# SuwoongHeo/neurecon

Hardware: AMD Instinct MI355X
Metric: rays/sec (4096 rays x 128 samples, 8-layer x256 SDF MLP) (higher is better)
Workload: dtype f16x3

## Files before the change

### include/neurecon_hip.h

```cpp
#ifndef NEURECON_HIP_H
#define NEURECON_HIP_H

#include <stddef.h>
#include <stdint.h>

#ifdef __cplusplus
extern "C" {
#endif

#define NR_OK 0
#define NR_ERR_ARG (-1)
#define NR_ERR_UNSUPPORTED (-2)
#define NR_ERR_HIP (-3)
#define NR_ERR_WORKSPACE (-4)

#define NR_PREC_FP32 0
#define NR_PREC_F16X3 1

#define NR_UPSAMPLE_OFFICIAL 0
#define NR_UPSAMPLE_DIRECT_USE 1
#define NR_UPSAMPLE_DIRECT_MORE 2

int nr_version(void);
const char* nr_last_error(void);
// ... 17 lines not shown
typedef struct {
  int D;
  int W;
  int skip;
  int multires;
  int W_geo_feat;
  int precision;
  int siren;
} NrSdfDesc;

size_t nr_sdf_packed_bytes(const NrSdfDesc* d);
int nr_sdf_pack(const NrSdfDesc* d, const float* const* W, const float* const* b, void* packed, void* stream);
size_t nr_mlp_workspace_bytes(int with_backward);
int nr_sdf_forward(const NrSdfDesc* d, const void* packed, const float* pts, int64_t P, float* sdf, float* nabla,
                   float* feature, void* workspace, size_t workspace_bytes, void* stream);

typedef struct {
  int D;
  int W;
  int multires;
  int multires_view;
  int W_geo_feat;
  int precision;
  int no_view_dirs;
  int siren;
} NrRadDesc;

size_t nr_radiance_packed_bytes(const NrRadDesc* d);
int nr_radiance_pack(const NrRadDesc* d, const float* const* W, const float* const* b, void* packed, void* stream);
int nr_radiance_forward(const NrRadDesc* d, const void* packed, const float* x, const float* vdir, int64_t vdir_div,
                        const float* normals, const float* feature, int64_t P, float* rgb, void* stream);

typedef struct {
  const float* rays_o;
  const float* rays_d;
  int64_t n_rays;
  const NrSdfDesc* sdf;
  const void* sdf_packed;
  const NrRadDesc* rad;
  const void* rad_packed;
  float s;
  float obj_bounding_radius;
  float near_bypass;
  float far_bypass;
  int N_samples;
  int N_importance;
  int N_upsample_iters;
  int calc_normal;
  int white_bkgd;
  const float* t_coarse;
  const float* u_fine;
  float* rgb;
  float* depth;
  float* acc;
  float* normals;
  float* d_final;
  float* sdf_out;
  float* nablas_out;
  float* radiance_out;
  float* alpha_out;
  float* cdf_out;
  float* weights_out;
  const NrNerfDesc* nerf;
  const void* nerf_packed;
  int N_outside;
  const float* t_outside;
  float* sigma_out;
  float* radiance_bg_out;
  int upsample_algo;
  float fixed_s;
  int N_nograd_samples;
  const float* t_nograd;
  void* workspace;
  size_t workspace_bytes;
  const float* u_rand;
  const float* t_out_rand;
  const float* s_dev;
  int sample_only;
  float* d_all_out;
  int no_mid_skip;
  int no_defer;
  int64_t max_chunk_rays;
  size_t max_workspace_bytes;
} NrNeusArgs;

#define NR_DEFAULT_WORKSPACE_BYTES ((size_t)4 << 30)
#define NR_MIN_CHUNK_RAYS 4096

size_t nr_neus_workspace_bytes(const NrNeusArgs* a);
int nr_neus_render(const NrNeusArgs* a, void* stream);

typedef struct {
  const float* rays_o;
  const float* rays_d;
  int64_t n_rays;
  const NrSdfDesc* sdf;
  const void* sdf_packed;
  const NrRadDesc* rad;
  const void* rad_packed;
  float alpha_net, beta_net;
  float beta_plus_init;
  float eps;
  float near, far;
  float obj_bounding_radius;
  int use_sphere_bg;
  int N_samples, N_importance, max_upsample_steps, max_bisection_steps;
  int calc_normal, white_bkgd;
  const float* t_coarse;
  const float* t_init;
  const float* u_up;
  const float* u_fine;
  float* rgb;
  float* depth;
  float* acc;
  float* normals;
  float* d_vals;
  float* sdf_out;
  float* nablas_out;
  float* radiance_out;
  float* alpha_out;
  float* p_out;
  float* weights_out;
  float* sigma_out;
  float* beta_map;
  float* iter_usage;
  void* workspace;
  size_t workspace_bytes;
  int N_outside;
  const NrNerfDesc* nerf;
  const void* nerf_packed;
  const float* rs_out;
  float beta_plus_k;
  float* sigma_bg;
  float* radiance_bg;
  const float* u_rand;
  const float* u_out;
} NrVolsdfArgs;

size_t nr_volsdf_workspace_bytes(const NrVolsdfArgs* a);
int nr_volsdf_render(const NrVolsdfArgs* a, void* stream);

typedef struct {
  const float* rays_o;
  const float* rays_d;
  int64_t n_rays;
  int64_t rays_per_batch;
  const NrSdfDesc* sdf;
  const void* sdf_packed;
  const NrRadDesc* rad;
  const void* rad_packed;
  float logit_tau;
  float radius_of_interest;
  float interval;
  float too_close_threshold;
  float near_bypass, far_bypass;
  int N_steps, N_secant_steps, N_query, N_freespace;
  int normal_mode;
  int64_t rayschunk, netchunk;
  int calc_normal, white_bkgd;
  const float* t_march;
  const float* t_query;
  const float* t_free;
  float* rgb;
  float* depth;
  float* acc;
  float* normals;
  float* surface_points;
  uint8_t* mask_surface;
  float* depth_surface;
  float* radiance_out;
  float* sdf_out;
  float* nablas_out;
  float* alpha_out;
// ... 265 lines not shown
```

### neurecon_amd/_lib.py

```python
import ctypes
import os
import threading

import torch

HERE = os.path.dirname(os.path.abspath(__file__))
LIB_PATH = os.environ.get('NR_LIB', os.path.join(HERE, 'libnrhip.so'))

PREC_FP32 = 0
PREC_F16X3 = 1
UPSAMPLE = {'official_solution': 0, 'direct_use': 1, 'direct_more': 2}

_c_p = ctypes.c_void_p
_c_i = ctypes.c_int
_c_i64 = ctypes.c_int64
_c_f = ctypes.c_float
_c_d = ctypes.c_double
_c_sz = ctypes.c_size_t


class NrSdfDesc(ctypes.Structure):
    _fields_ = [('D', _c_i), ('W', _c_i), ('skip', _c_i), ('multires', _c_i), ('W_geo_feat', _c_i),
                ('precision', _c_i), ('siren', _c_i)]


class NrRadDesc(ctypes.Structure):
    _fields_ = [('D', _c_i), ('W', _c_i), ('multires', _c_i), ('multires_view', _c_i), ('W_geo_feat', _c_i),
                ('precision', _c_i), ('no_view_dirs', _c_i), ('siren', _c_i)]


class NrNerfDesc(ctypes.Structure):
    _fields_ = [('D', _c_i), ('W', _c_i), ('skip', _c_i), ('input_ch', _c_i), ('multires', _c_i),
                ('multires_view', _c_i), ('precision', _c_i)]


class NrNeusArgs(ctypes.Structure):
    _fields_ = [
        ('rays_o', _c_p), ('rays_d', _c_p), ('n_rays', _c_i64),
        ('sdf', ctypes.POINTER(NrSdfDesc)), ('sdf_packed', _c_p),
        ('rad', ctypes.POINTER(NrRadDesc)), ('rad_packed', _c_p),
        ('s', _c_f), ('obj_bounding_radius', _c_f), ('near_bypass', _c_f), ('far_bypass', _c_f),
        ('N_samples', _c_i), ('N_importance', _c_i), ('N_upsample_iters', _c_i), ('calc_normal', _c_i),
        ('white_bkgd', _c_i),
        ('t_coarse', _c_p), ('u_fine', _c_p),
        ('rgb', _c_p), ('depth', _c_p), ('acc', _c_p), ('normals', _c_p),
        ('d_final', _c_p), ('sdf_out', _c_p), ('nablas_out', _c_p), ('radiance_out', _c_p),
        ('alpha_out', _c_p), ('cdf_out', _c_p), ('weights_out', _c_p),
        ('nerf', ctypes.POINTER(NrNerfDesc)), ('nerf_packed', _c_p), ('N_outside', _c_i), ('t_outside', _c_p),
        ('sigma_out', _c_p), ('radiance_bg_out', _c_p),
        ('upsample_algo', _c_i), ('fixed_s', _c_f), ('N_nograd_samples', _c_i), ('t_nograd', _c_p),
        ('workspace', _c_p), ('workspace_bytes', _c_sz),
        ('u_rand', _c_p), ('t_out_rand', _c_p), ('s_dev', _c_p), ('sample_only', _c_i), ('d_all_out', _c_p),
        ('no_mid_skip', _c_i), ('no_defer', _c_i), ('max_chunk_rays', _c_i64), ('max_workspace_bytes', _c_sz),
    ]


class NrVolsdfArgs(ctypes.Structure):
    _fields_ = [
        ('rays_o', _c_p), ('rays_d', _c_p), ('n_rays', _c_i64),
        ('sdf', ctypes.POINTER(NrSdfDesc)), ('sdf_packed', _c_p),
        ('rad', ctypes.POINTER(NrRadDesc)), ('rad_packed', _c_p),
        ('alpha_net', _c_f), ('beta_net', _c_f), ('beta_plus_init', _c_f), ('eps', _c_f),
        ('near', _c_f), ('far', _c_f), ('obj_bounding_radius', _c_f), ('use_sphere_bg', _c_i),
        ('N_samples', _c_i), ('N_importance', _c_i), ('max_upsample_steps', _c_i), ('max_bisection_steps', _c_i),
        ('calc_normal', _c_i), ('white_bkgd', _c_i),
        ('t_coarse', _c_p), ('t_init', _c_p), ('u_up', _c_p), ('u_fine', _c_p),
        ('rgb', _c_p), ('depth', _c_p), ('acc', _c_p), ('normals', _c_p),
        ('d_vals', _c_p), ('sdf_out', _c_p), ('nablas_out', _c_p), ('radiance_out', _c_p),
        ('alpha_out', _c_p), ('p_out', _c_p), ('weights_out', _c_p), ('sigma_out', _c_p),
        ('beta_map', _c_p), ('iter_usage', _c_p),
        ('workspace', _c_p), ('workspace_bytes', _c_sz),
        ('N_outside', _c_i), ('nerf', ctypes.POINTER(NrNerfDesc)), ('nerf_packed', _c_p), ('rs_out', _c_p),
        ('beta_plus_k', _c_f), ('sigma_bg', _c_p), ('radiance_bg', _c_p), ('u_rand', _c_p), ('u_out', _c_p),
    ]


class NrUnisurfArgs(ctypes.Structure):
    _fields_ = [
        ('rays_o', _c_p), ('rays_d', _c_p), ('n_rays', _c_i64), ('rays_per_batch', _c_i64),
        ('sdf', ctypes.POINTER(NrSdfDesc)), ('sdf_packed', _c_p),
        ('rad', ctypes.POINTER(NrRadDesc)), ('rad_packed', _c_p),
        ('logit_tau', _c_f), ('radius_of_interest', _c_f), ('interval', _c_f), ('too_close_threshold', _c_f),
        ('near_bypass', _c_f), ('far_bypass', _c_f),
        ('N_steps', _c_i), ('N_secant_steps', _c_i), ('N_query', _c_i), ('N_freespace', _c_i),
        ('normal_mode', _c_i), ('rayschunk', _c_i64), ('netchunk', _c_i64),
        ('calc_normal', _c_i), ('white_bkgd', _c_i),
        ('t_march', _c_p), ('t_query', _c_p), ('t_free', _c_p),
        ('rgb', _c_p), ('depth', _c_p), ('acc', _c_p), ('normals', _c_p),
        ('surface_points', _c_p), ('mask_surface', _c_p), ('depth_surface', _c_p),
        ('radiance_out', _c_p), ('sdf_out', _c_p), ('nablas_out', _c_p), ('alpha_out', _c_p), ('weights_out', _c_p),
        ('workspace', _c_p), ('workspace_bytes', _c_sz),
        ('u_query', _c_p), ('u_free', _c_p),
        ('shard_ray0', _c_i64), ('shard_row_rays', _c_i64), ('window_ss', _c_p), ('window_reduce', _c_p),
        ('window_user', _c_p), ('no_secant', _c_i), ('d_all_out', _c_p), ('sample_only', _c_i),
        ('full_march', _c_i),
    ]


WINDOW_REDUCE = ctypes.CFUNCTYPE(_c_i, _c_p)

TG_NONE, TG_SOFTPLUS, TG_MUL, TG_SPADJ, TG_RELUMASK = 0, 1, 3, 4, 5
BLK_X1, BLK_X2, BLK_Y, BLK_YB, BLK_Y2, BLK_Y3, BLK_A, BLK_G, BLK_ZD = 1, 2, 4, 8, 16, 32, 64, 128, 256
WG_BLK_A0, WG_BLK_A1, WG_BLK_B0, WG_BLK_B1 = 1, 2, 4, 8
WN_MAX = 16
ADAM_MAX = 64


class NrTrainGemm(ctypes.Structure):
    _fields_ = [
        ('op', _c_p), ('P', _c_i64),
        ('x1', _c_p), ('ld1', _c_i64), ('n1', _c_i),
        ('x2', _c_p), ('ld2', _c_i64), ('n2', _c_i),
        ('use_bias', _c_i), ('mode', _c_i), ('yscale', _c_f),
        ('y', _c_p), ('ldy', _c_i64), ('yb', _c_p), ('ldyb', _c_i64),
        ('y2', _c_p), ('ldy2', _c_i64), ('y3', _c_p), ('ldy3', _c_i64),
        ('a', _c_p), ('lda', _c_i64), ('g', _c_p), ('ldg', _c_i64), ('zd', _c_p), ('ldzd', _c_i64),
        ('g_row', _c_i), ('dot', _c_p), ('dot_bias', _c_f),
        ('head', _c_p), ('head_bias', _c_p), ('head_out', _c_p), ('blocked', _c_i),
        ('g_scaled', _c_i),
    ]


class NrWgrad(ctypes.Structure):
    _fields_ = [
        ('P', _c_i64), ('npairs', _c_i), ('a', _c_p * 2), ('lda', _c_i64 * 2), ('b', _c_p * 2), ('ldb', _c_i64 * 2),
        ('m', _c_i), ('n', _c_i), ('scale', _c_f), ('c', _c_p), ('ldc', _c_i64), ('colsum', _c_p),
        ('avec', _c_p), ('ldv', _c_i64), ('vec', _c_p), ('vec_scale', _c_f), ('workspace', _c_p),
        ('workspace_bytes', _c_sz), ('blocked', _c_i), ('fp32', _c_i),
    ]


class NrWnLayer(ctypes.Structure):
    _fields_ = [('v', _c_p), ('g', _c_p), ('w', _c_p), ('norm', _c_p), ('grad_w', _c_p), ('grad_v', _c_p),
                ('grad_g', _c_p), ('rows', _c_i), ('cols', _c_i)]


class NrAdamTensor(ctypes.Structure):
    _fields_ = [('param', _c_p), ('grad', _c_p), ('exp_avg', _c_p), ('exp_avg_sq', _c_p), ('n', _c_i64)]


class NrKernelStat(ctypes.Structure):
    _fields_ = [('name', ctypes.c_char * 32), ('launches', _c_i64), ('ms', ctypes.c_double),
                ('units', ctypes.c_double)]


_SIGS = {
    'nr_version': (_c_i, []),
    'nr_last_error': (ctypes.c_char_p, []),
    'nr_build_id': (ctypes.c_char_p, []),
    'nr_sdf_packed_bytes': (_c_sz, [ctypes.POINTER(NrSdfDesc)]),
    'nr_sdf_pack': (_c_i, [ctypes.POINTER(NrSdfDesc), ctypes.POINTER(_c_p), ctypes.POINTER(_c_p), _c_p, _c_p]),
    'nr_mlp_workspace_bytes': (_c_sz, [_c_i]),
    'nr_sdf_forward': (_c_i, [ctypes.POINTER(NrSdfDesc), _c_p, _c_p, _c_i64, _c_p, _c_p, _c_p, _c_p, _c_sz, _c_p]),
    'nr_radiance_packed_bytes': (_c_sz, [ctypes.POINTER(NrRadDesc)]),
    'nr_radiance_pack': (_c_i, [ctypes.POINTER(NrRadDesc), ctypes.POINTER(_c_p), ctypes.POINTER(_c_p), _c_p, _c_p]),
    'nr_radiance_forward': (_c_i, [ctypes.POINTER(NrRadDesc), _c_p, _c_p, _c_p, _c_i64, _c_p, _c_p, _c_i64, _c_p,
                                   _c_p]),
    'nr_nerf_packed_bytes': (_c_sz, [ctypes.POINTER(NrNerfDesc)]),
    'nr_nerf_pack': (_c_i, [ctypes.POINTER(NrNerfDesc), ctypes.POINTER(_c_p), ctypes.POINTER(_c_p), _c_p, _c_p]),
    'nr_nerf_forward': (_c_i, [ctypes.POINTER(NrNerfDesc), _c_p, _c_p, _c_p, _c_i64, _c_i64, _c_p, _c_p, _c_p]),
    'nr_nerf_train_fwd32': (_c_i, [ctypes.POINTER(NrNerfDesc), _c_p, _c_p, _c_p, _c_i64, ctypes.POINTER(_c_p), _c_p,
                                   _c_p, _c_p, _c_p, _c_p]),
    'nr_nerf_train_packed_bytes': (_c_sz, [ctypes.POINTER(NrNerfDesc)]),
    'nr_weight_norm_fwd': (_c_i, [ctypes.POINTER(NrWnLayer), _c_i, _c_p]),
    'nr_weight_norm_bwd': (_c_i, [ctypes.POINTER(NrWnLayer), _c_i, _c_p]),
    'nr_adam_step': (_c_i, [ctypes.POINTER(NrAdamTensor), _c_i, _c_i64, _c_d, _c_d, _c_d, _c_d, _c_d, _c_p]),
    'nr_nerf_train_pack': (_c_i, [ctypes.POINTER(NrNerfDesc), ctypes.POINTER(_c_p), ctypes.POINTER(_c_p), _c_p, _c_p]),
    'nr_nerf_train_bwd32': (_c_i, [ctypes.POINTER(NrNerfDesc), _c_p, _c_p, _c_p, ctypes.POINTER(_c_p), _c_p, _c_p,
                                   _c_i64, _c_p, _c_p, _c_p, ctypes.POINTER(_c_p), _c_p]),
    'nr_neus_workspace_bytes': (_c_sz, [ctypes.POINTER(NrNeusArgs)]),
    'nr_neus_render': (_c_i, [ctypes.POINTER(NrNeusArgs), _c_p]),
    'nr_volsdf_workspace_bytes': (_c_sz, [ctypes.POINTER(NrVolsdfArgs)]),
    'nr_volsdf_render': (_c_i, [ctypes.POINTER(NrVolsdfArgs), _c_p]),
    'nr_unisurf_workspace_bytes': (_c_sz, [ctypes.POINTER(NrUnisurfArgs)]),
    'nr_unisurf_render': (_c_i, [ctypes.POINTER(NrUnisurfArgs), _c_p]),
    'nr_unisurf_window_count': (_c_i64, [ctypes.POINTER(NrUnisurfArgs)]),
    'nr_sample_pdf': (_c_i, [_c_p, _c_p, _c_i64, _c_i, _c_p, _c_i64, _c_i, _c_p, _c_p]),
    'nr_get_rays': (_c_i, [_c_p, _c_p, _c_i, _c_i, _c_i, _c_p, _c_i64, _c_p, _c_p, _c_p]),
    'nr_gather_rows': (_c_i, [_c_p, _c_i64, _c_i64, _c_i64, _c_p, _c_i64, _c_p, _c_p]),
    'nr_sphere_trace_workspace_bytes': (_c_sz, [_c_i64]),
    'nr_sphere_trace': (_c_i, [ctypes.POINTER(NrSdfDesc), _c_p, _c_p, _c_p, _c_i64, ctypes.c_float, ctypes.c_float,
                               _c_p, _c_p, _c_i, _c_p, _c_p, _c_p, _c_p, _c_sz, _c_p]),
    'nr_radiance_train_fwd32': (_c_i, [ctypes.POINTER(NrRadDesc), _c_p, _c_p, _c_p, _c_i64, _c_i64, _c_p, _c_p, _c_p,
                                        _c_p, _c_p, _c_p]),
    'nr_root_find_workspace_bytes': (_c_sz, [_c_i64, _c_i]),
    'nr_root_find': (_c_i, [ctypes.POINTER(NrSdfDesc), _c_p, _c_p, _c_p, _c_i64, ctypes.c_float, ctypes.c_float, _c_p,
                            _c_p, _c_i, _c_p, _c_i, _c_i, ctypes.c_float, _c_i, _c_i, _c_p, _c_p, _c_p, _c_p, _c_p,
                            _c_sz, _c_p]),
    'nr_normalize3': (_c_i, [_c_p, _c_i64, _c_p, _c_p]),
    'nr_surface_finish': (_c_i, [_c_p, _c_p, _c_p, _c_i64, _c_p, _c_p]),
    'nr_sdf_grid_workspace_bytes': (_c_sz, [_c_i64]),
    'nr_sdf_grid': (_c_i, [ctypes.POINTER(NrSdfDesc), _c_p, ctypes.c_double, _c_i64, _c_i64, _c_i64, _c_p, _c_p,
                           _c_sz, _c_p]),
    'nr_embed': (_c_i, [_c_p, _c_i64, _c_i, _c_p, _c_p]),
    'nr_embed_jvp': (_c_i, [_c_p, _c_p, _c_i64, _c_i, _c_p, _c_p]),
    'nr_embed_vjp': (_c_i, [_c_p, _c_p, _c_i, _c_p, _c_i, _c_f, _c_i64, _c_i, _c_p, _c_p]),
    'nr_embed_padded': (_c_i, [_c_p, _c_i64, _c_i, _c_p, _c_i, _c_p]),
    'nr_embed_jvp_padded': (_c_i, [_c_p, _c_p, _c_i64, _c_i, _c_p, _c_i, _c_p]),
    'nr_train_gemm': (_c_i, [ctypes.POINTER(NrTrainGemm), _c_i, _c_i, _c_i, _c_i, _c_p]),
    'nr_sdf_op_info': (_c_i, [ctypes.POINTER(NrSdfDesc), _c_i, ctypes.POINTER(_c_i64), ctypes.POINTER(_c_i),
                              ctypes.POINTER(_c_i)]),
    'nr_sdf_train_packed_bytes': (_c_sz, [ctypes.POINTER(NrSdfDesc)]),
    'nr_sdf_train_pack': (_c_i, [ctypes.POINTER(NrSdfDesc), ctypes.POINTER(_c_p), ctypes.POINTER(_c_p), _c_p, _c_p]),
    'nr_radiance_op_info': (_c_i, [ctypes.POINTER(NrRadDesc), _c_i, ctypes.POINTER(_c_i64), ctypes.POINTER(_c_i),
                                   ctypes.POINTER(_c_i)]),
    'nr_radiance_train_packed_bytes': (_c_sz, [ctypes.POINTER(NrRadDesc)]),
    'nr_radiance_train_pack': (_c_i, [ctypes.POINTER(NrRadDesc), ctypes.POINTER(_c_p), ctypes.POINTER(_c_p), _c_p,
                                      _c_p]),
    'nr_softplus100': (_c_i, [_c_p, _c_i64, _c_p, _c_p, _c_p]),
    'nr_scale_cols': (_c_i, [_c_p, _c_i64, _c_i, _c_i, _c_i, _c_p, _c_f, _c_p, _c_p]),
    'nr_softplus_adjoint': (_c_i, [_c_p, _c_i, _c_p, _c_p, _c_p, _c_i64, _c_i, _c_p, _c_p]),
    'nr_colsum_workspace_bytes': (_c_sz, [_c_i]),
    'nr_colsum': (_c_i, [_c_p, _c_i64, _c_i, _c_p, _c_p, _c_sz, _c_p]),
    'nr_sine30': (_c_i, [_c_p, _c_i64, _c_p, _c_p, _c_p]),
    'nr_sine_adjoint': (_c_i, [_c_p, _c_i, _c_p, _c_p, _c_p, _c_p, _c_i64, _c_i, _c_p, _c_p]),
    'nr_mul': (_c_i, [_c_p, _c_p, _c_i64, _c_p, _c_p]),
    'nr_activation': (_c_i, [_c_p, _c_p, _c_i64, _c_i, _c_p]),
    'nr_radiance_input': (_c_i, [_c_p, _c_p, _c_p, _c_p, _c_i64, _c_i, _c_i, _c_i, _c_p, _c_p]),
    'nr_neus_points': (_c_i, [_c_p, _c_p, _c_p, _c_i64, _c_i, _c_p, _c_p, _c_p, _c_p]),
    'nr_neus_composite_fwd': (_c_i, [_c_p, _c_p, _c_p, _c_p, _c_i64, _c_i, _c_i, _c_p, _c_p, _c_p, _c_p, _c_p, _c_p,
                                     _c_p]),
    'nr_neus_composite_bwd_workspace_bytes': (_c_sz, [_c_i64, _c_i]),
    'nr_neus_composite_bwd': (_c_i, [_c_p, _c_p, _c_p, _c_p, _c_i64, _c_i, _c_i, _c_p, _c_p, _c_p, _c_p, _c_p, _c_p,
                                     _c_p, _c_p, _c_sz, _c_p]),
    'nr_nerf_train_input': (_c_i, [_c_p, _c_p, _c_p, _c_i64, _c_i, _c_i, ctypes.c_float, _c_p, _c_p, _c_p, _c_p]),
    'nr_neus_composite_bg_fwd': (_c_i, [_c_p, _c_p, _c_p, _c_p, _c_p, _c_p, _c_p, _c_i64, _c_i, _c_i, _c_i, _c_p, _c_p,
                                        _c_p, _c_p, _c_p, _c_p, _c_p]),
    'nr_neus_composite_bg_bwd_workspace_bytes': (_c_sz, [_c_i64, _c_i, _c_i]),
    'nr_neus_composite_bg_bwd': (_c_i, [_c_p, _c_p, _c_p, _c_p, _c_p, _c_p, _c_p, _c_i64, _c_i, _c_i, _c_i, _c_p, _c_p,
                                        _c_p, _c_p, _c_p, _c_p, _c_p, _c_p, _c_p, _c_p, _c_sz, _c_p]),
    'nr_unisurf_composite_fwd': (_c_i, [_c_p, _c_p, _c_p, _c_i64, _c_i, _c_i, _c_p, _c_p, _c_p, _c_p, _c_p, _c_p]),
    'nr_unisurf_composite_bwd_workspace_bytes': (_c_sz, [_c_i64, _c_i]),
    'nr_unisurf_composite_bwd': (_c_i, [_c_p, _c_p, _c_p, _c_i64, _c_i, _c_i, _c_p, _c_p, _c_p, _c_p, _c_p, _c_p, _c_p,
                                        _c_sz, _c_p]),
    'nr_volsdf_composite_bg_fwd': (_c_i, [_c_p, _c_p, _c_p, _c_p, _c_p, _c_i64, _c_i, _c_i, _c_f, _c_i, _c_p, _c_p,
                                          _c_p, _c_i, _c_p, _c_p, _c_p, _c_p, _c_p, _c_p, _c_p, _c_p]),
    'nr_volsdf_composite_bg_bwd_workspace_bytes': (_c_sz, [_c_i64, _c_i, _c_i]),
    'nr_volsdf_composite_bg_bwd': (_c_i, [_c_p, _c_p, _c_p, _c_p, _c_p, _c_i64, _c_i, _c_i, _c_f, _c_i, _c_p, _c_p,
                                          _c_p, _c_i, _c_p, _c_p, _c_p, _c_p, _c_p, _c_p, _c_p, _c_p, _c_p, _c_p, _c_p,
                                          _c_sz, _c_p]),
    'nr_volsdf_nerf_input': (_c_i, [_c_p, _c_p, _c_p, _c_p, _c_i64, _c_i, _c_p, _c_p, _c_p]),
    'nr_volsdf_composite_fwd': (_c_i, [_c_p, _c_p, _c_p, _c_p, _c_p, _c_i64, _c_i, _c_i, _c_f, _c_i, _c_p, _c_p, _c_p,
                                       _c_p, _c_p, _c_p, _c_p, _c_p]),
    'nr_volsdf_composite_bwd_workspace_bytes': (_c_sz, [_c_i64, _c_i]),
    'nr_volsdf_composite_bwd': (_c_i, [_c_p, _c_p, _c_p, _c_p, _c_p, _c_i64, _c_i, _c_i, _c_f, _c_i, _c_p, _c_p, _c_p,
                                       _c_p, _c_p, _c_p, _c_p, _c_p, _c_p, _c_sz, _c_p]),
    'nr_wgrad_workspace_bytes': (_c_sz, [_c_i64, _c_i, _c_i, _c_i]),
    'nr_wgrad': (_c_i, [ctypes.POINTER(NrWgrad), _c_p]),
    'nr_profile_enable': (_c_i, [_c_i]),
    'nr_gemm32': (_c_i, [_c_p, _c_i64, _c_p, _c_i64, _c_i, _c_p, _c_p, _c_i64, _c_i64, _c_i, _c_i, _c_i, _c_p]),
    'nr_profile_filter': (_c_i, [ctypes.c_char_p]),
    'nr_profile_read': (_c_i, [ctypes.POINTER(NrKernelStat), _c_i, ctypes.POINTER(_c_i)]),
}

# ... 86 lines not shown
```

### neurecon_amd/base.py

```python
import math

import numpy as np
import torch
import torch.nn as nn
import torch.nn.functional as F

from . import _lib as L


class Embedder(nn.Module):
    def __init__(self, input_dim, max_freq_log2, N_freqs, log_sampling=True, include_input=True,
                 periodic_fns=(torch.sin, torch.cos)):
        super().__init__()
        self.input_dim = input_dim
        self.include_input = include_input
        self.periodic_fns = periodic_fns
        self.out_dim = (input_dim if include_input else 0) + input_dim * N_freqs * len(periodic_fns)
        bands = 2. ** torch.linspace(0., max_freq_log2, N_freqs) if log_sampling else \
            torch.linspace(2. ** 0., 2. ** max_freq_log2, N_freqs)
        self.freq_bands = bands.numpy().tolist()

    def forward(self, x):
        assert x.shape[-1] == self.input_dim
        parts = [x] if self.include_input else []
# ... 210 lines not shown

    def forward(self, x, return_h=False):
        sdf, _, h = self._run(x, nabla=False, feature=return_h)
        return (sdf, h) if return_h else sdf

    def forward_with_nablas(self, x, has_grad_bypass=None):
        sdf, nab, h = self._run(x, nabla=True, feature=True)
        return sdf, nab, h

    def pretrain_hook(self, configs={}):
        configs['target_radius'] = self.radius_init
        configs['obj_bounding_size'] = float(self.obj_bounding_size.reshape(-1)[0])
        if self.geometric_init and self.use_siren and not bool(self.is_pretrained):
            pretrain_siren_sdf(self, **configs)
            self.is_pretrained = ~self.is_pretrained
            return True
        return False


def pretrain_siren_sdf(implicit_surface, num_iters=5000, lr=1.0e-4, batch_points=5000, target_radius=0.5,
                       obj_bounding_size=3.0, logger=None):
    from torch import optim
    device = next(implicit_surface.parameters()).device
    optimizer = optim.Adam(implicit_surface.parameters(), lr=lr)
    with torch.enable_grad():
        for it in range(num_iters):
            pts = torch.empty([batch_points, 3]).uniform_(-obj_bounding_size, obj_bounding_size).float().to(device)
            sdf_gt = pts.norm(dim=-1) - target_radius
            sdf_pred = implicit_surface.forward(pts)
            loss = F.l1_loss(sdf_pred, sdf_gt, reduction='mean')
            optimizer.zero_grad()
            loss.backward()
            optimizer.step()
            if logger is not None:
                logger.add('pretrain_siren', 'loss_l1', loss.item(), it)


class RadianceNet(nn.Module):

    def __init__(self, D=4, W=256, skips=[], W_geo_feat=256, embed_multires=6, embed_multires_view=4,
                 use_view_dirs=True, weight_norm=True, use_siren=False, precision=None):
        super().__init__()
        if not weight_norm or skips:
            raise NotImplementedError('neurecon_amd: RadianceNet needs weight_norm and no skips')
        self.D, self.W, self.skips, self.use_view_dirs = D, W, list(skips), bool(use_view_dirs)
        self.use_siren = bool(use_siren)
        self.embed_multires, self.embed_multires_view, self.W_geo_feat = embed_multires, embed_multires_view, W_geo_feat
        self.embed_fn, ch_pts = get_embedder(embed_multires)
        if use_view_dirs:
            self.embed_fn_view, ch_view = get_embedder(embed_multires_view)
            in0 = ch_pts + ch_view + 3 + W_geo_feat
        else:
            in0 = ch_pts + W_geo_feat
        self.precision = default_precision() if precision is None else precision
        self.layers = nn.ModuleList([
            WNLinear(in0 if l == 0 else W, W, *_siren_init(in0 if l == 0 else W, W, l == 0))
            if use_siren and l != D else WNLinear(in0 if l == 0 else W, 3 if l == D else W) for l in range(D + 1)])
        self._nr_cache = None

    def nr_desc(self):
        return L.NrRadDesc(self.D, self.W, self.embed_multires, self.embed_multires_view, self.W_geo_feat,
                           L.PREC_FP32 if self.precision == 'fp32' else L.PREC_F16X3, 0 if self.use_view_dirs else 1,
                           1 if self.use_siren else 0)

    def nr_packed(self, device):
        key = _version_key(self, self.precision, device)
        if self._nr_cache is not None and self._nr_cache[0] == key:
            return self._nr_cache[1], self._nr_cache[2]
        lib = L.lib()
        desc = self.nr_desc()
        nbytes = lib.nr_radiance_packed_bytes(ctypes.byref(desc))
        if nbytes == 0:
            raise NotImplementedError('neurecon_amd: ' + lib.nr_last_error().decode())
        with torch.no_grad():
            Ws, bs = _wn_params(self.layers)
            Ws = [w.to(device) for w in Ws]
            bs = [b.to(device) for b in bs]
            packed = torch.empty(nbytes, dtype=torch.uint8, device=device)
            L.check(lib.nr_radiance_pack(ctypes.byref(desc), _ptr_array(Ws), _ptr_array(bs), L.ptr(packed),
                                         L.stream_of(device)))
        self._nr_cache = (key, desc, packed, Ws, bs)
        return desc, packed

    def forward(self, x, view_dirs, normals, geometry_feature):
        L.require_gpu(x, 'points')
        shape = x.shape[:-1]
        P = x.reshape(-1, 3).shape[0]
        if self.use_view_dirs:
            if view_dirs is None:
                raise TypeError('RadianceNet(use_view_dirs=True) needs view_dirs')
            v = view_dirs.reshape(-1, 3).float().contiguous()
            if v.shape[0] != P:
                raise ValueError('view_dirs must have one direction per point')
            n = normals.reshape(-1, 3).float().contiguous()
        else:
            v = n = None
        if wants_graph(self, normals, geometry_feature):
            from .training import radiance
            rgb = radiance(self, x.reshape(-1, 3).float(), v, n, geometry_feature.reshape(-1, self.W_geo_feat).float())
            return rgb.reshape(*shape, 3)
        dev = x.device
        xs = x.reshape(-1, 3).float().contiguous()
        f = geometry_feature.reshape(-1, self.W_geo_feat).float().contiguous()
        desc, packed = self.nr_packed(dev)
        rgb = torch.empty(P, 3, device=dev)
        L.check(L.lib().nr_radiance_forward(ctypes.byref(desc), L.ptr(packed), L.ptr(xs), L.ptr(v), 1, L.ptr(n),
                                            L.ptr(f), P, L.ptr(rgb), L.stream_of(dev)))
        return rgb.reshape(*shape, 3)


class NeRF(nn.Module):
    def __init__(self, D=8, W=256, input_ch=3, input_ch_view=3, multires=-1, multires_view=-1, output_ch=4,
                 skips=[4], use_view_dirs=False, precision=None):
        super().__init__()
        self.D, self.W, self.skips, self.use_view_dirs = D, W, list(skips), use_view_dirs
        self.multires, self.multires_view, self.input_ch_raw = multires, multires_view, input_ch
        self.embed_fn, input_ch = get_embedder(multires, input_dim=input_ch)
        self.embed_fn_view, input_ch_view = get_embedder(multires_view, input_dim=input_ch_view)
        self.pts_linears = nn.ModuleList(
            [nn.Linear(input_ch, W)] + [nn.Linear(W + input_ch if i in self.skips else W, W) for i in range(D - 1)])
        self.views_linears = nn.ModuleList([nn.Linear(input_ch_view + W, W // 2)])
        if use_view_dirs:
            self.feature_linear = nn.Linear(W, W)
            self.alpha_linear = nn.Linear(W, 1)
            self.rgb_linear = nn.Linear(W // 2, 3)
        else:
            self.output_linear = nn.Linear(W, output_ch)
        self.precision = default_precision() if precision is None else precision
        self._nr_cache = None

    def nr_desc(self):
        if not self.use_view_dirs or len(self.skips) != 1:
            raise NotImplementedError('neurecon_amd: only the NeRF++ background configuration is native')
        return L.NrNerfDesc(self.D, self.W, self.skips[0], self.input_ch_raw, self.multires, self.multires_view,
                            L.PREC_FP32 if self.precision == 'fp32' else L.PREC_F16X3)

    def nr_packed(self, device):
        key = _version_key(self, self.precision, device)
        if self._nr_cache is not None and self._nr_cache[0] == key:
            return self._nr_cache[1], self._nr_cache[2]
        lib = L.lib()
        desc = self.nr_desc()
        nbytes = lib.nr_nerf_packed_bytes(ctypes.byref(desc))
        if nbytes == 0:
            raise NotImplementedError('neurecon_amd: ' + lib.nr_last_error().decode())
        layers = list(self.pts_linears) + [self.feature_linear, self.views_linears[0], self.alpha_linear,
                                           self.rgb_linear]
        with torch.no_grad():
            Ws = [l.weight.detach().float().contiguous().to(device) for l in layers]
            bs = [l.bias.detach().float().contiguous().to(device) for l in layers]
            packed = torch.empty(nbytes, dtype=torch.uint8, device=device)
            L.check(lib.nr_nerf_pack(ctypes.byref(desc), _ptr_array(Ws), _ptr_array(bs), L.ptr(packed),
                                     L.stream_of(device)))
        self._nr_cache = (key, desc, packed, Ws, bs)
        return desc, packed

    def forward(self, input_pts, input_views):
        L.require_gpu(input_pts, 'points')
        _no_training(self, what='the NeRF++ background net')
        shape = input_pts.shape[:-1]
        dev = input_pts.device
        x = input_pts.reshape(-1, 4).float().contiguous()
        P = x.shape[0]
        v = input_views.reshape(-1, 3).float().contiguous()
        if v.shape[0] != P:
            raise ValueError('input_views must have one direction per point')
# ... 7 lines not shown
```

### neurecon_amd/csrc/nr_capi.hip

```cpp
#include <algorithm>
#include <cmath>
#include <cstring>
#include <string>

#include "nr_common.h"
#include <cstdlib>
#include "nr_mlp.h"
#include "nr_tgemm.h"
#include "nr_neus.h"
#include "nr_volsdf.h"
#include "nr_unisurf.h"

namespace nr {

static thread_local std::string g_err;
void set_error(const std::string& msg) { g_err = msg; }

static size_t align256(size_t x) { return (x + 255) & ~(size_t)255; }
static int64_t chunk_bytes_host(int KB) { return (int64_t)(2 * KB + 1) * 1024; }

int check_sdf_desc(const NrSdfDesc* d) {
  NR_REQUIRE(d, NR_ERR_ARG, "null NrSdfDesc");
  if (d->siren) {
    NR_REQUIRE(d->D == 5 && d->W == 256 && d->skip < 0 && d->multires < 0 && d->W_geo_feat == 256,
               NR_ERR_UNSUPPORTED,
               "SIREN SDF net: only D=5, W=256, skips=[], embed_multires=-1, W_geo_feat=256 (configs/volsdf_siren.yaml)");
    NR_REQUIRE(d->precision == NR_PREC_FP32 || d->precision == NR_PREC_F16X3, NR_ERR_UNSUPPORTED,
               "SDF net: unknown precision mode");
    return NR_OK;
  }
  NR_REQUIRE(d->D == 8 && d->W == 256 && d->skip == 4 && d->multires == 6 && d->W_geo_feat == 256,
             NR_ERR_UNSUPPORTED,
             "SDF net: only D=8, W=256, skips=[4], embed_multires=6, W_geo_feat=256 are implemented");
  NR_REQUIRE(d->precision == NR_PREC_FP32 || d->precision == NR_PREC_F16X3, NR_ERR_UNSUPPORTED,
             "SDF net: unknown precision mode");
  return NR_OK;
}

int check_rad_desc(const NrRadDesc* d) {
  NR_REQUIRE(d, NR_ERR_ARG, "null NrRadDesc");
  NR_REQUIRE((d->D == 4 || d->D == 5) && d->W == 256 && d->multires < 0 && d->W_geo_feat == 256 &&
                 d->multires_view <= 7,
             NR_ERR_UNSUPPORTED,
             "radiance net: only D=4 or 5, W=256, embed_multires=-1, embed_multires_view<=7, W_geo_feat=256");
  NR_REQUIRE(d->precision == NR_PREC_FP32 || d->precision == NR_PREC_F16X3, NR_ERR_UNSUPPORTED,
             "radiance net: unknown precision mode");
  return NR_OK;
}


SdfLayout sdf_layout(const NrSdfDesc& d) {
  SdfLayout L{};
  L.prec = d.precision;
  L.siren = d.siren ? 1 : 0;
  const int nops = L.siren ? kSirenOps : kSdfOps;
  const int* KB = L.siren ? kSirenKB : kSdfKB;
  const int* NBO = L.siren ? kSirenNBO : kSdfNBO;
  size_t off = 0;
  for (int i = 0; i < nops; ++i) {
    L.op_bytes[i] = (2 * KB[i] + 1) * 1024;
    L.op_off[i] = (uint32_t)off;
    off += (size_t)(NBO[i] / 2) * L.op_bytes[i];
  }
  static_assert(sdf_op_off(kSdfOps - 1) + (kSdfNBO[kSdfOps - 1] / 2) * (2 * kSdfKB[kSdfOps - 1] + 1) * 1024 > 0, "");
  L.scale_off = (uint32_t)off;
  off = align256(off + kSdfOps * 4);
  L.bound_off = (uint32_t)off;
  off = align256(off + kSdfOps * 8);
  L.w8row0_off = (uint32_t)off;
  off = align256(off + 256 * 4);
  L.misc_off = (uint32_t)off;
  off = align256(off + 16);
  L.total = (uint32_t)off;
  return L;
}

static int rad_small(const NrRadDesc& d) {
  return d.no_view_dirs ? 3 : 3 + (d.multires_view < 0 ? 3 : 3 + 6 * d.multires_view) + 3;
}

RadLayout rad_layout(const NrRadDesc& d) {
  RadLayout L{};
  L.prec = d.precision;
  L.n_small = rad_small(d);
  L.view = d.no_view_dirs ? 0 : 1;
  L.D = d.D;
  L.siren = d.siren ? 1 : 0;
  L.kbs = L.n_small <= 32 ? 2 : 4;
  size_t off = 0;
  for (int i = 0; i < L.D; ++i) {
    const int kb = i == 0 ? 16 + L.kbs : 16;
    L.op_bytes[i] = (2 * kb + 1) * 1024;
    L.op_off[i] = (uint32_t)off;
    off += 8 * (size_t)L.op_bytes[i];
  }
  L.scale_off = (uint32_t)off;
  off = align256(off + 5 * 4);
  L.bound_off = (uint32_t)off;
  off = align256(off + 5 * 2 * 4);
  L.head_off = (uint32_t)off;
  off = align256(off + (3 * 256 + 4) * 4);
  L.total = (uint32_t)off;
  return L;
}

int check_nerf_desc(const NrNerfDesc* d) {
  NR_REQUIRE(d, NR_ERR_ARG, "null NrNerfDesc");
  NR_REQUIRE(d->D == 8 && d->W == 256 && d->skip == 4 && d->input_ch == 4 && d->multires == 10 &&
                 d->multires_view == 4,
             NR_ERR_UNSUPPORTED,
             "NeRF net: only the NeRF++ background configuration (D=8, W=256, skips=[4], input_ch=4, "
             "multires=10, multires_view=4, use_view_dirs) is implemented");
  NR_REQUIRE(d->precision == NR_PREC_FP32 || d->precision == NR_PREC_F16X3, NR_ERR_UNSUPPORTED,
             "NeRF net: unknown precision mode");
  return NR_OK;
}

static const int kNerfKB[kNerfOps] = {6, 16, 16, 16, 16, 22, 16, 16, 16, 18};
static const int kNerfNBO[kNerfOps] = {16, 16, 16, 16, 16, 16, 16, 16, 16, 8};

static int nerf_nbo(int i, int prec) { return (i == NF && prec == NR_PREC_F16X3) ? 18 : kNerfNBO[i]; }

NerfLayout nerf_layout(const NrNerfDesc& d) {
  NerfLayout L{};
  L.prec = d.precision;
  size_t off = 0;
  for (int i = 0; i < kNerfOps; ++i) {
    L.op_bytes[i] = (2 * kNerfKB[i] + 1) * 1024;
    L.op_off[i] = (uint32_t)off;
    off += (size_t)(nerf_nbo(i, d.precision) / 2) * L.op_bytes[i];
  }
  L.scale_off = (uint32_t)off;
  off = align256(off + kNerfOps * 4);
  L.bound_off = (uint32_t)off;
  off = align256(off + kNerfOps * 2 * 4);
  L.alpha_off = (uint32_t)off;
  off = align256(off + 257 * 4);
  L.rgb_off = (uint32_t)off;
  off = align256(off + (3 * 128 + 3) * 4);
  L.total = (uint32_t)off;
  return L;
}

static PackSeg seg(int nblk, int off, int nvalid) { return PackSeg{nblk, off, nvalid}; }
static PackOp mkop(const float* W, const float* bias, int rows, int ld, int tr, PackSeg o0, PackSeg o1, PackSeg i0,
                   PackSeg i1, float scale, int prec, float* wmax) {
  PackOp op{};
  op.W = W; op.bias = bias; op.wn = (int64_t)rows * ld; op.ld = ld; op.transpose = tr;
  op.out[0] = o0; op.out[1] = o1; op.in[0] = i0; op.in[1] = i1;
  op.scale = scale; op.prec = prec; op.wmax = wmax;
  return op;
}
static PackSeg none() { return PackSeg{0, 0, 0}; }

static size_t scratch_bytes() {
  int dev = 0, cus = 256;
  if (hipGetDevice(&dev) == hipSuccess) (void)hipDeviceGetAttribute(&cus, hipDeviceAttributeMultiprocessorCount, dev);
  return (size_t)cus * kScratchPerWG;
}

static int neus_chunk(const NrNeusArgs& a, const NeusPlan& pl, int64_t ray0, int R, hipStream_t st) {
  char* ws = (char*)a.workspace;
  const bool direct = a.upsample_algo != NR_UPSAMPLE_OFFICIAL;
  const int n_up = direct ? 0 : (a.N_upsample_iters > 0 ? a.N_importance / a.N_upsample_iters : 0);
  NeusChunk c{};
  c.R = R;
  c.N_samples = a.N_samples;
  c.n_up = n_up;
  c.n_iters = direct ? 0 : a.N_upsample_iters;
  c.S = direct ? a.N_samples + a.N_importance : a.N_samples + a.N_upsample_iters * n_up;
  c.n_imp = a.N_importance;
  c.n_nog = a.upsample_algo == NR_UPSAMPLE_DIRECT_MORE ? a.N_nograd_samples : 0;
  c.fixed_s = a.fixed_s;
  c.t_nog = a.t_nograd;
  auto F = [&](size_t o) { return (float*)(ws + o); };
  c.ro = F(pl.o_ro); c.rd = F(pl.o_rd); c.near = F(pl.o_near); c.far = F(pl.o_far);
  c.dv = F(pl.o_dv); c.sv = F(pl.o_sv); c.wtmp = F(pl.o_wtmp); c.dnew = F(pl.o_dnew); c.snew = F(pl.o_snew);
  c.pts = F(pl.o_pts); c.mids = F(pl.o_mids); c.dmid = F(pl.o_dmid);
  c.sdf_f = F(pl.o_sdf_f); c.nab_f = F(pl.o_nab_f);
  c.sdf_m = F(pl.o_sdf_m); c.nab_m = F(pl.o_nab_m); c.feat_m = F(pl.o_feat_m); c.rad_m = F(pl.o_rad_m);
  c.N_out = a.N_outside;
  c.r_obj = a.obj_bounding_radius;
  c.t_out = a.t_outside;
  c.d_out = F(pl.o_dout); c.x4 = F(pl.o_x4); c.sig_o = F(pl.o_sigo); c.rad_o = F(pl.o_rado);
  c.pts_nog = F(pl.o_ptsn); c.s_nog = F(pl.o_sn);
  const bool fused = !direct && !a.sample_only;
// ... 37 lines not shown
    hipLaunchKernelGGL(neus_nograd_points, grd, blk, 0, st, c);
    NR_HIP_CHECK(hipGetLastError());
    if ((rc = launch_sdf(SL, a.sdf_packed, c.pts_nog, (int64_t)c.n_nog * R, c.s_nog, nullptr, nullptr,
                         a.sdf->multires, nullptr, 0, st)))
      return rc;
  }
  if (direct) {
    ProfScope prof("neus_upsample", (double)R, st);
    const float* u = a.u_rand ? a.u_rand + ray0 * a.N_importance : a.u_fine;
    hipLaunchKernelGGL(neus_direct_upsample, grd, blk, 0, st, c, (int)(a.upsample_algo == NR_UPSAMPLE_DIRECT_MORE), u,
                       (int64_t)(a.u_rand ? a.N_importance : 0));
  }
  NR_HIP_CHECK(hipGetLastError());
  float* dvb[2] = {c.dv, F(pl.o_dv2)};
  float* svb[2] = {c.sv, F(pl.o_sv2)};
  int* idb[2] = {c.idv, fused ? (int*)(ws + pl.o_idv2) : nullptr};
  int cur = 0;
  auto merge = [&](int L) -> int {
    ProfScope prof("neus_merge", (double)R, st);
    const int64_t nt = (int64_t)(L + n_up) * R;
    hipLaunchKernelGGL(neus_merge, dim3((unsigned)((nt + 255) / 256)), dim3(256), 0, st, c, L, dvb[cur ^ 1],
                       svb[cur ^ 1], idb[cur ^ 1]);
    cur ^= 1;
    c.dv = dvb[cur];
    c.sv = svb[cur];
    c.idv = idb[cur];
    if (fused) c.sdf_f = c.sv;
    NR_HIP_CHECK(hipGetLastError());
    return NR_OK;
  };
  for (int it = 0; it < c.n_iters; ++it) {
    if (it > 0 && (rc = merge(a.N_samples + (it - 1) * n_up))) return rc;
    const int64_t slot0 = (int64_t)(a.N_samples + it * n_up) * R;
    NeusChunk cu = c;
    if (defer) cu.pts = c.pts + slot0 * 3;
    {
      ProfScope prof("neus_upsample", (double)R, st);
      const float* u = a.u_rand ? a.u_rand + ((int64_t)it * a.n_rays + ray0) * n_up : a.u_fine;
      const size_t lds1 = (5 * (size_t)c.S + 1) * sizeof(float);
      if (4 * lds1 <= 65536)
        hipLaunchKernelGGL((neus_upsample<4>), dim3((unsigned)((R + 3) / 4)), dim3(64), 4 * lds1, st, cu, it, u,
                           (int64_t)(a.u_rand ? n_up : 0));
      else
        hipLaunchKernelGGL((neus_upsample<1>), dim3((unsigned)R), dim3(64), lds1, st, cu, it, u,
                           (int64_t)(a.u_rand ? n_up : 0));
    }
    NR_HIP_CHECK(hipGetLastError());
    if ((rc = sample_sdf(cu.pts, (int64_t)n_up * R, c.snew, slot0))) return rc;
  }
  if (c.n_iters > 0 && (rc = merge(c.S - n_up))) return rc;
  if (defer) {
    const int64_t nslot = (int64_t)c.S * R;
    c.tshift = 0;
    NR_HIP_CHECK(hipMemsetAsync(c.nraw, 0, (size_t)nslot * 3 * sizeof(float), st));
    if (a.calc_normal && a.N_outside == 0) {
      NR_HIP_CHECK(hipMemsetAsync(c.tflag, 0, (size_t)nslot * sizeof(int), st));
      NR_HIP_CHECK(hipMemsetAsync(c.tcnt, 0, sizeof(int), st));
      const int64_t nq = (int64_t)(c.S - 1) * R;
      hipLaunchKernelGGL(neus_sample_need, dim3((unsigned)((nq + 255) / 256)), dim3(256), 0, st, c, a.s_dev, a.s);
      NR_HIP_CHECK(hipGetLastError());
      hipLaunchKernelGGL(neus_point_list, dim3((unsigned)((nslot + 1023) / 1024)), dim3(1024), 0, st, c, nslot);
      NR_HIP_CHECK(hipGetLastError());
      if ((rc = launch_sdf_deferred(SL, a.sdf_packed, c.pts, nslot, nullptr, c.nraw, a.sdf->multires, c.slabs, c.tiles,
                                    c.tcnt, 4, st)))
        return rc;
    }
  }
  if (a.sample_only) {
    hipLaunchKernelGGL(neus_write_dall, dim3((unsigned)(((int64_t)c.S * R + 255) / 256)), dim3(256), 0, st, c.dv,
                       (int64_t)R, c.S, ray0, a.d_all_out);
    NR_HIP_CHECK(hipGetLastError());
    return NR_OK;
  }
  {
    ProfScope prof("neus_points", (double)R, st);
    hipLaunchKernelGGL(neus_expand, dim3((unsigned)(((int64_t)c.S * R + 255) / 256)), dim3(256), 0, st, c,
                       (int)!(defer && a.N_outside > 0));
  }
  NR_HIP_CHECK(hipGetLastError());
  if (!fused && (rc = launch_sdf(SL, a.sdf_packed, c.pts, (int64_t)c.S * R, c.sdf_f, c.nab_f, nullptr,
                                 a.sdf->multires, mlp_ws, mlp_bytes, st)))
    return rc;
  const int64_t Pm = (int64_t)(c.S - 1) * R;
  if (a.radiance_out || a.no_mid_skip) {
    if ((rc = launch_sdf(SL, a.sdf_packed, c.mids, Pm, c.sdf_m, c.nab_m, c.feat_m, a.sdf->multires, mlp_ws, mlp_bytes,
                         st)))
      return rc;
    if ((rc = launch_radiance(RL, a.rad_packed, c.mids, c.rd, 1, R, c.nab_m, c.feat_m, Pm, c.rad_m,
                              a.rad->multires_view, st)))
      return rc;
  } else {
    char* wsb = (char*)a.workspace;
    int* cnt = (int*)(wsb + pl.o_mcnt);
    int* slot = (int*)(wsb + pl.o_mslot);
    float* midc = (float*)(wsb + pl.o_midc);
    float* vdc = (float*)(wsb + pl.o_mvd);
    float* radc = (float*)(wsb + pl.o_mrad);
    NR_HIP_CHECK(hipMemsetAsync(cnt, 0, sizeof(int), st));
    const dim3 g1((unsigned)((Pm + 255) / 256));
    hipLaunchKernelGGL(neus_mid_compact, dim3((unsigned)((Pm + 1023) / 1024)), dim3(1024), 0, st, c, a.s_dev, a.s, cnt,
                       slot, midc, vdc);
    NR_HIP_CHECK(hipGetLastError());
    if ((rc = launch_sdf(SL, a.sdf_packed, midc, Pm, c.sdf_m, c.nab_m, c.feat_m, a.sdf->multires, mlp_ws, mlp_bytes,
                         st, cnt, 1)))
      return rc;
    if ((rc = launch_radiance(RL, a.rad_packed, midc, vdc, 1, INT64_MAX, c.nab_m, c.feat_m, Pm, radc,
                              a.rad->multires_view, st, cnt)))
      return rc;
    hipLaunchKernelGGL(neus_mid_scatter, g1, dim3(256), 0, st, slot, radc, Pm, c.rad_m);
    NR_HIP_CHECK(hipGetLastError());
  }
  NeusOut o{ray0, a.rgb, a.depth, a.acc, a.normals, a.d_final, a.sdf_out, a.nablas_out,
            a.radiance_out, a.alpha_out, a.cdf_out, a.weights_out, a.sigma_out, a.radiance_bg_out};
  if (a.N_outside > 0) {
    hipLaunchKernelGGL(neus_outside_points, grd, blk, 0, st, c,
                       a.t_out_rand ? a.t_out_rand + ray0 * a.N_outside : (const float*)nullptr);
    NR_HIP_CHECK(hipGetLastError());
    const int64_t Po = (int64_t)(c.S - 1 + a.N_outside) * R;
    if (a.sigma_out || a.radiance_bg_out) {
      if ((rc = launch_nerf(nerf_layout(*a.nerf), a.nerf_packed, c.x4, c.rd, 1, R, Po, c.sig_o, c.rad_o, st)))
        return rc;
    } else {
      char* wsb = (char*)a.workspace;
      int* cnt = (int*)(wsb + pl.o_cnt);
      int* slot = (int*)(wsb + pl.o_slot);
      float* x4c = (float*)(wsb + pl.o_x4c);
      float* vdc = (float*)(wsb + pl.o_vdc);
      float* sigc = (float*)(wsb + pl.o_sigc);
      float* radc = (float*)(wsb + pl.o_radc);
      NR_HIP_CHECK(hipMemsetAsync(cnt, 0, sizeof(int), st));
      const dim3 g1((unsigned)((Po + 255) / 256));
      hipLaunchKernelGGL(neus_outside_compact, dim3((unsigned)((Po + 1023) / 1024)), dim3(1024), 0, st, c, cnt, slot,
                         x4c, vdc);
      NR_HIP_CHECK(hipGetLastError());
      if ((rc = launch_nerf(nerf_layout(*a.nerf), a.nerf_packed, x4c, vdc, 1, INT64_MAX, Po, sigc, radc, st, cnt)))
        return rc;
      hipLaunchKernelGGL(neus_outside_scatter, g1, dim3(256), 0, st, slot, sigc, radc, Po, c.sig_o, c.rad_o);
      NR_HIP_CHECK(hipGetLastError());
    }
    if (defer) {
      const int64_t nslot = (int64_t)c.S * R;
      c.tshift = 0;
      if (a.calc_normal) {
        NR_HIP_CHECK(hipMemsetAsync(c.tflag, 0, (size_t)nslot * sizeof(int), st));
        NR_HIP_CHECK(hipMemsetAsync(c.tcnt, 0, sizeof(int), st));
        hipLaunchKernelGGL(neus_sample_need_outside, dim3((unsigned)((nslot + 255) / 256)), dim3(256), 0, st, c,
                           a.s_dev, a.s);
        NR_HIP_CHECK(hipGetLastError());
        hipLaunchKernelGGL(neus_point_list, dim3((unsigned)((nslot + 1023) / 1024)), dim3(1024), 0, st, c, nslot);
        NR_HIP_CHECK(hipGetLastError());
        if ((rc = launch_sdf_deferred(SL, a.sdf_packed, c.pts, nslot, nullptr, c.nraw, a.sdf->multires, c.slabs,
                                      c.tiles, c.tcnt, 4, st)))
          return rc;
      }
      hipLaunchKernelGGL(neus_gather_nablas, dim3((unsigned)((nslot + 255) / 256)), dim3(256), 0, st, c);
      NR_HIP_CHECK(hipGetLastError());
    }
    ProfScope prof("neus_composite", (double)R, st);
    const int M = c.S - 1 + a.N_outside;
    const size_t lds1 = (6 * (size_t)M + 4 * (size_t)c.S) * sizeof(float);
    if (4 * lds1 <= 65536)
      hipLaunchKernelGGL((neus_composite_outside_w<4>), dim3((unsigned)((R + 3) / 4)), dim3(64), 4 * lds1, st, c, o,
                         a.s_dev, a.s, a.calc_normal, a.white_bkgd);
    else if (lds1 <= 65536)
      hipLaunchKernelGGL((neus_composite_outside_w<1>), dim3((unsigned)R), dim3(64), lds1, st, c, o, a.s_dev, a.s,
                         a.calc_normal, a.white_bkgd);
    else
      hipLaunchKernelGGL(neus_composite_outside, grd, blk, 0, st, c, o, a.s_dev, a.s, a.calc_normal, a.white_bkgd);
  } else {
    ProfScope prof("neus_composite", (double)R, st);
    const size_t lds1 = 9 * (size_t)c.S * sizeof(float);
    if (4 * lds1 <= 65536)
      hipLaunchKernelGGL((neus_composite<4>), dim3((unsigned)((R + 3) / 4)), dim3(64), 4 * lds1, st, c, o, a.s_dev, a.s,
                         a.calc_normal, a.white_bkgd);
    else
      hipLaunchKernelGGL((neus_composite<1>), dim3((unsigned)R), dim3(64), lds1, st, c, o, a.s_dev, a.s, a.calc_normal,
                         a.white_bkgd);
  }
  NR_HIP_CHECK(hipGetLastError());
  return NR_OK;
}

static int64_t neus_chunk_rays(const NrNeusArgs* a) {
  const int64_t n = a->n_rays > 0 ? a->n_rays : 1;
  int64_t cap = 16384;
  if (a->max_chunk_rays > 0)
    cap = std::min(cap, a->max_workspace_bytes ? a->max_chunk_rays : std::max<int64_t>(a->max_chunk_rays, NR_MIN_CHUNK_RAYS));
  const size_t budget = a->max_workspace_bytes ? a->max_workspace_bytes : NR_DEFAULT_WORKSPACE_BYTES;
  const bool defer = neus_deferred(*a, 16);
  NrNeusArgs q = *a;
// ... 611 lines not shown
  return NR_OK;
}

static void rad_train_layout(const RadLayout& L, int64_t (&off)[5], int (&kb)[5], int (&nbo)[5], int64_t& total) {
  const int KBs[5] = {2, 16, 16, 16, 16};
  const int NBOs[5] = {16, 16, 16, 16, 16 + L.kbs};
  int64_t o = 0;
  for (int i = 0; i < 5; ++i) {
    off[i] = o; kb[i] = KBs[i]; nbo[i] = NBOs[i];
    o += (int64_t)(NBOs[i] / 2) * chunk_bytes_host(KBs[i]);
  }
  total = o;
}

int nr_radiance_op_info(const NrRadDesc* d, int op, int64_t* offset, int* kb, int* nbo) {
  int rc = train_radiance(d);
  if (rc) return rc;
  NR_REQUIRE(offset && kb && nbo && op >= 0 && op <= 2 * d->D + 1, NR_ERR_ARG, "nr_radiance_op_info: bad argument");
  const RadLayout L = rad_layout(*d);
  if (op < d->D) {
    *offset = L.op_off[op]; *kb = op == 0 ? 16 + L.kbs : 16; *nbo = 16;
  } else if (op == d->D) {
    *offset = L.head_off; *kb = 0; *nbo = 0;
  } else {
    int64_t off[5], total;
    int kbs[5], nbos[5];
    rad_train_layout(L, off, kbs, nbos, total);
    const int i = op - d->D - 1;
    *offset = off[i]; *kb = kbs[i]; *nbo = nbos[i];
  }
  return NR_OK;
}

size_t nr_radiance_train_packed_bytes(const NrRadDesc* d) {
  if (train_radiance(d)) return 0;
  int64_t off[5], total;
  int kb[5], nbo[5];
  rad_train_layout(rad_layout(*d), off, kb, nbo, total);
  return align256((size_t)total + 5 * 4) + 256;
}

int nr_radiance_train_pack(const NrRadDesc* d, const float* const* W, const float* const* b, void* packed,
                           void* stream) {
  int rc = train_radiance(d);
  if (rc) return rc;
  NR_REQUIRE(W && b && packed, NR_ERR_ARG, "nr_radiance_train_pack: null argument");
  for (int l = 0; l <= d->D; ++l) NR_REQUIRE(W[l], NR_ERR_ARG, "nr_radiance_train_pack: null layer pointer");
  hipStream_t st = (hipStream_t)stream;
  const RadLayout L = rad_layout(*d);
  int64_t off[5], total;
  int kb[5], nbo[5];
  rad_train_layout(L, off, kb, nbo, total);
  char* P = (char*)packed;
  float* wmax = (float*)(P + total);
  const int ns = L.n_small, ld0 = ns + 256;
  PackOp ops[5];
  ops[0] = mkop(W[4], nullptr, 3, 256, 1, seg(16, 0, 256), none(), seg(2, 0, 3), none(), 1.0f, NR_PREC_F16X3, wmax);
  for (int i = 1; i <= 3; ++i)
    ops[i] = mkop(W[4 - i], nullptr, 256, 256, 1, seg(16, 0, 256), none(), seg(16, 0, 256), none(), 1.0f,
                  NR_PREC_F16X3, wmax + i);
  ops[4] = mkop(W[0], nullptr, 256, ld0, 1, seg(16, ns, 256), seg(L.kbs, 0, ns), seg(16, 0, 256), none(), 1.0f,
                NR_PREC_F16X3, wmax + 4);
  char* dst[5];
  for (int i = 0; i < 5; ++i) dst[i] = P + off[i];
  if ((rc = launch_pack_ops(ops, dst, 5, st))) return rc;
  return NR_OK;
}

size_t nr_neus_workspace_bytes(const NrNeusArgs* a) {
  if (!a) return 0;
  return neus_plan(*a, neus_chunk_rays(a)).total;
}

int nr_neus_render(const NrNeusArgs* a, void* stream) {
  NR_REQUIRE(a, NR_ERR_ARG, "nr_neus_render: null args");
  int rc = check_sdf_desc(a->sdf);
  if (rc) return rc;
  if ((rc = check_rad_desc(a->rad))) return rc;
  NR_REQUIRE(a->n_rays <= 0 || (a->rays_o && a->rays_d && (a->sample_only ? a->d_all_out != nullptr
                                                                            : (a->rgb && a->depth && a->acc))),
             NR_ERR_ARG, "nr_neus_render: null ray or output pointer");
  NR_REQUIRE(a->sdf_packed && a->rad && (a->rad_packed || a->sample_only) && a->t_coarse, NR_ERR_ARG,
             "nr_neus_render: null argument");
  NR_REQUIRE(a->N_samples >= 2, NR_ERR_ARG, "nr_neus_render: N_samples must be >= 2");
  NR_REQUIRE(a->n_rays <= 0 || a->sample_only || !a->calc_normal || a->normals, NR_ERR_ARG,
             "nr_neus_render: calc_normal needs normals output");
  NR_REQUIRE(a->N_outside >= 0, NR_ERR_ARG, "nr_neus_render: N_outside must be >= 0");
  if (a->N_outside > 0) {
    if ((rc = check_nerf_desc(a->nerf))) return rc;
    NR_REQUIRE(a->nerf_packed && a->t_outside, NR_ERR_ARG, "nr_neus_render: N_outside > 0 needs the NeRF++ net");
  }
  NR_REQUIRE(a->upsample_algo >= NR_UPSAMPLE_OFFICIAL && a->upsample_algo <= NR_UPSAMPLE_DIRECT_MORE, NR_ERR_ARG,
             "nr_neus_render: unknown upsample_algo");
  if (a->upsample_algo != NR_UPSAMPLE_OFFICIAL) {
    NR_REQUIRE(a->N_importance >= 1 && a->u_fine && a->fixed_s > 0.f, NR_ERR_ARG,
               "nr_neus_render: direct upsampling needs N_importance >= 1, u_fine and fixed_s > 0");
    NR_REQUIRE(a->upsample_algo != NR_UPSAMPLE_DIRECT_MORE || (a->N_nograd_samples >= 2 && a->t_nograd), NR_ERR_ARG,
               "nr_neus_render: direct_more needs N_nograd_samples >= 2 and t_nograd");
  } else if (a->N_upsample_iters > 0) {
    const int n_up = a->N_importance / a->N_upsample_iters;
    NR_REQUIRE(n_up >= 1 && n_up <= kMaxUp && a->u_fine, NR_ERR_UNSUPPORTED,
               "nr_neus_render: N_importance/N_upsample_iters must be in [1, 32]");
  }
  if (a->n_rays <= 0) return NR_OK;
  const int64_t Rc = neus_chunk_rays(a);
  const NeusPlan pl = neus_plan(*a, Rc);
  NR_REQUIRE(a->workspace && a->workspace_bytes >= pl.total, NR_ERR_WORKSPACE, "nr_neus_render: workspace too small");
  {
    const bool direct = a->upsample_algo != NR_UPSAMPLE_OFFICIAL;
    const int S = direct ? a->N_samples + a->N_importance
                         : a->N_samples + a->N_upsample_iters * (a->N_upsample_iters > 0 ? a->N_importance / a->N_upsample_iters : 0);
    int dev = 0, lds_max = 65536;
    NR_HIP_CHECK(hipGetDevice(&dev));
    NR_HIP_CHECK(hipDeviceGetAttribute(&lds_max, hipDeviceAttributeMaxSharedMemoryPerBlock, dev));
    NR_REQUIRE((size_t)9 * S * sizeof(float) <= (size_t)lds_max, NR_ERR_UNSUPPORTED,
               "nr_neus_render: N_samples + N_importance too large for the per-ray LDS staging of the compositing");
  }
  for (int64_t r0 = 0; r0 < a->n_rays; r0 += Rc) {
    const int R = (int)((a->n_rays - r0) < Rc ? (a->n_rays - r0) : Rc);
    if ((rc = neus_chunk(*a, pl, r0, R, (hipStream_t)stream))) return rc;
  }
  return NR_OK;
}

size_t nr_volsdf_workspace_bytes(const NrVolsdfArgs* a) {
  if (!a || check_volsdf(a)) return 0;
  return volsdf_plan(*a, volsdf_chunk_rays(a)).total;
}

int nr_volsdf_render(const NrVolsdfArgs* a, void* stream) {
  int rc = check_volsdf(a);
  if (rc) return rc;
  if (a->n_rays <= 0) return NR_OK;
  const int64_t Rc = volsdf_chunk_rays(a);
  const VolPlan pl = volsdf_plan(*a, Rc);
  NR_REQUIRE(a->workspace && a->workspace_bytes >= pl.total, NR_ERR_WORKSPACE,
             "nr_volsdf_render: workspace too small");
  int dev = 0, lds_max = 65536;
  NR_HIP_CHECK(hipGetDevice(&dev));
  NR_HIP_CHECK(hipDeviceGetAttribute(&lds_max, hipDeviceAttributeMaxSharedMemoryPerBlock, dev));
  NR_REQUIRE(pl.lds_bytes <= (size_t)lds_max, NR_ERR_UNSUPPORTED,
             "nr_volsdf_render: per-ray sample list does not fit in LDS (reduce N_samples or max_upsample_steps)");
  for (int64_t r0 = 0; r0 < a->n_rays; r0 += Rc) {
    const int R = (int)((a->n_rays - r0) < Rc ? (a->n_rays - r0) : Rc);
    if ((rc = volsdf_chunk(*a, pl, r0, R, (hipStream_t)stream))) return rc;
  }
  return NR_OK;
}

size_t nr_unisurf_workspace_bytes(const NrUnisurfArgs* a) {
  if (!a || check_unisurf(a)) return 0;
  return unisurf_plan(*a, unisurf_chunk_rays(*a)).total;
}

int64_t nr_unisurf_window_count(const NrUnisurfArgs* a) {
  if (!a || a->normal_mode != 1) return 0;
  int64_t rc_rays, nw_full, nw_row;
  unisurf_windows(*a, rc_rays, nw_full, nw_row);
  return nw_row;
}

int nr_unisurf_render(const NrUnisurfArgs* a, void* stream) {
  int rc = check_unisurf(a);
  if (rc) return rc;
  const bool sharded = a->shard_row_rays > 0;
  if (a->n_rays <= 0) {
    if (sharded) NR_REQUIRE(a->window_reduce(a->window_user) == 0, NR_ERR_ARG, "nr_unisurf_render: window_reduce failed");
    return NR_OK;
  }
  const int64_t Rc = unisurf_chunk_rays(*a);
  const UniPlan pl = unisurf_plan(*a, Rc);
  NR_REQUIRE(a->workspace && a->workspace_bytes >= pl.total, NR_ERR_WORKSPACE,
             "nr_unisurf_render: workspace too small");
  if (sharded)
    return unisurf_chunk(*a, pl, 0, (int)a->n_rays, a->shard_ray0,
                         (int)(a->rays_per_batch > 0 ? a->rays_per_batch : a->n_rays), (hipStream_t)stream);
  const int64_t per_b = (a->normal_mode == 1 && a->rays_per_batch > 0) ? a->rays_per_batch : a->n_rays;
  const int64_t span = a->normal_mode == 1 ? (a->rayschunk < per_b ? a->rayschunk : per_b) : per_b;
  for (int64_t b0 = 0; b0 < a->n_rays; b0 += per_b) {
    const int64_t b1 = b0 + per_b < a->n_rays ? b0 + per_b : a->n_rays;
    for (int64_t c0 = b0; c0 < b1; c0 += span) {
      const int64_t c1 = c0 + span < b1 ? c0 + span : b1;
      for (int64_t r0 = c0; r0 < c1; r0 += Rc) {
        const int R = (int)((c1 - r0) < Rc ? (c1 - r0) : Rc);
        if ((rc = unisurf_chunk(*a, pl, r0, R, r0 - b0, R, (hipStream_t)stream))) return rc;
      }
    }
  }
  return NR_OK;
}

int nr_sample_pdf(const float* bins, const float* weights, int64_t R, int L, const float* u, int64_t u_stride, int N,
                  float* out, void* stream) {
  NR_REQUIRE(bins && weights && u && out && L >= 2 && N >= 1 && u_stride >= 0, NR_ERR_ARG,
             "nr_sample_pdf: bad argument");
  if (R <= 0) return NR_OK;
  hipLaunchKernelGGL(sample_pdf_kernel, dim3((unsigned)((R + 255) / 256)), dim3(256), 0, (hipStream_t)stream, bins,
                     weights, R, L, u, u_stride, N, out);
  NR_HIP_CHECK(hipGetLastError());
  return NR_OK;
}

}
```

### neurecon_amd/csrc/nr_mlp.h

```cpp
#pragma once
#include "nr_common.h"

namespace nr {

constexpr int kWaves = 8;
constexpr int kThreads = 64 * kWaves;
constexpr int kTile = 16;
constexpr int kPointsPerWG = kTile * kWaves;
constexpr int kMaxChunkBytes = 48 * 1024;
constexpr size_t kScratchPerWG = (size_t)kWaves * 8 * 16 * 64 * 16;
constexpr int kSlabVB = 12;
constexpr int kSlab24Chunk = 2 * 64 * kSlabVB;
constexpr int kSlab24Layer = 8 * kSlab24Chunk;
constexpr int kSlabColBytes = 7 * kSlab24Layer + 16 * 64 * 16;

enum SdfOp { F0, F1, F2, F3, F4, F5, F6, F7, F8, B7, B6, B5, B4, B3, B2, B1, B0, kSdfOps };

constexpr int kSdfKB[kSdfOps] = {4, 16, 16, 16, 18, 16, 16, 16, 16, 16, 16, 16, 16, 14, 16, 16, 16};
constexpr int kSdfNBO[kSdfOps] = {16, 16, 16, 14, 16, 16, 16, 16, 16, 16, 16, 16, 18, 16, 16, 16, 4};
__host__ __device__ constexpr uint32_t sdf_op_off(int i) {
  uint32_t off = 0;
  for (int k = 0; k < i; ++k) off += (uint32_t)(kSdfNBO[k] / 2) * (2 * kSdfKB[k] + 1) * 1024;
  return off;
}
// ... 4 lines not shown
static_assert(kSirenOps <= kSdfOps, "SIREN ops share SdfLayout's offset table");

struct SdfLayout {
  uint32_t op_off[kSdfOps];
  uint32_t op_bytes[kSdfOps];
  uint32_t scale_off;
  uint32_t bound_off;
  uint32_t w8row0_off;
  uint32_t misc_off;
  uint32_t total;
  int prec;
  int siren;
};

struct RadLayout {
  uint32_t op_off[5];
  uint32_t op_bytes[5];
  uint32_t head_off;
  uint32_t scale_off;
  uint32_t bound_off;
  uint32_t total;
  int prec;
  int kbs;
  int n_small;
  int view;
  int D;
  int siren;
};

enum NerfOp { N0, N1, N2, N3, N4, N5, N6, N7, NF, NV, kNerfOps };

struct NerfLayout {
  uint32_t op_off[kNerfOps];
  uint32_t op_bytes[kNerfOps];
  uint32_t scale_off;
  uint32_t bound_off;
  uint32_t alpha_off;
  uint32_t rgb_off;
  uint32_t total;
  int prec;
};

enum NerfBwdOp { NBV, NBF, NB7, NB6, NB5, NB4, NB3, NB2, NB1, kNerfBwdOps };

struct NerfBwdLayout {
  uint32_t op_off[kNerfBwdOps];
  uint32_t op_bytes[kNerfBwdOps];
  uint32_t scale_off;
  uint32_t wr_off;
  uint32_t wa_off;
  uint32_t total;
};

struct PackSeg {
  int nblk;
  int off;
  int nvalid;
};

struct PackOp {
  const float* W;
  const float* bias;
  int64_t wn;
  int ld;
  int transpose;
  PackSeg out[2];
  PackSeg in[2];
  float scale;
  int prec;
  float* wmax;
  const float* aux;
  float* bound;
  const float* W2;
  const float* bias2;
  int64_t wn2;
  int ld2;
};

int launch_pack_op(const PackOp& op, char* dst, hipStream_t stream);
int launch_pack_ops(const PackOp* ops, char* const* dst, int nops, hipStream_t stream);
int launch_pack_vec(const float* src, int off, int nvalid, int n, char* dst, hipStream_t stream);
int launch_sdf(const SdfLayout& L, const void* packed, const float* pts, int64_t P, float* sdf, float* nabla,
               float* feature, int nfreq, void* ws, size_t ws_bytes, hipStream_t stream,
               const int* P_dev = nullptr, int P_mult = 0);
int launch_sdf_deferred(const SdfLayout& L, const void* packed, const float* pts, int64_t P, float* sdf, float* nabla,
                        int nfreq, float4* slabs, const int* tiles, const int* n_tiles, int stage, hipStream_t stream);
int launch_nerf(const NerfLayout& L, const void* packed, const float* x4, const float* vdir, int64_t vdiv,
                int64_t vmod, int64_t P, float* sigma, float* rgb, hipStream_t stream,
                const int* P_dev = nullptr);
int launch_radiance(const RadLayout& L, const void* packed, const float* x, const float* vdir, int64_t vdiv,
                    int64_t vmod, const float* normals, const float* feature, int64_t P, float* rgb, int nfreq_view,
                    hipStream_t stream, const int* P_dev = nullptr);

int launch_radiance_train32(const RadLayout& L, const void* packed, const float* feat, const float* small,
                            int64_t ld_small, int n_small, int64_t P, float* const* h, float* rgb, hipStream_t stream);
int launch_nerf_train32_fwd(const NerfLayout& L, const void* packed, const float* xe, const float* ve, int64_t P,
                            float* const* h, float* feat, float* hv, float* sigma, float* rgb, hipStream_t stream);
int launch_nerf_train32_bwd(const NerfBwdLayout& B, const void* packed, const float* rgb, const float* hv,
                            const float* const* h, const float* g_rgb, const float* g_sigma, int64_t P, float* g3,
                            float* ghv, float* g_feat, float* const* gz, hipStream_t stream,
                            bool f16x3 = false);
SdfLayout sdf_layout(const NrSdfDesc& d);
RadLayout rad_layout(const NrRadDesc& d);
int check_sdf_desc(const NrSdfDesc* d);
int check_rad_desc(const NrRadDesc* d);

}
```

### neurecon_amd/csrc/nr_mlp.hip

```cpp
#include <algorithm>
#include <type_traits>
#include "nr_common.h"
#include "nr_mlp.h"
#include "nr_tgemm.h"

namespace nr {

using lds_ptr = __attribute__((address_space(3))) void*;

__device__ __forceinline__ void glds16(const char* gsrc, uint32_t lds_addr) {
  unsigned keep;
  asm volatile(
      "s_mov_b32 %0, m0\n\t"
      "s_mov_b32 m0, %2\n\t"
      "s_nop 0\n\t"
      "global_load_lds_dwordx4 %1, off\n\t"
      "s_mov_b32 m0, %0"
      : "=&s"(keep)
      : "v"(gsrc), "s"(lds_addr)
      : "memory");
}

__device__ __forceinline__ void glds16s(const char* sbase, uint32_t voff, uint32_t lds_addr) {
  unsigned keep;
// ... 384 lines not shown
    else if (nxt) ws.issue(nxt + (c + 2 - NCH) * nxt_bytes, nxt_bytes);
    else ws.none();
    const float4* A = ws.buf();
    f32x4 acc0 = {0, 0, 0, 0}, acc1 = {0, 0, 0, 0};
    if constexpr (P == NR_PREC_FP32) {
      mma_chunk<KBG, 0, 4>(A, G, dummy, acc0, acc1, lane);
    } else {
      mma_chunk_h3<KBG / 2>(A, bh, bl, acc0, acc1, lane);
      const float inv = ginv * A[2 * KBG * 64 + 8].x;
      acc0 = acc0 * inv;
      acc1 = acc1 * inv;
    }
    float4 y0 = fromf(acc0), y1 = fromf(acc1);
    if (main) {
      if (e_cur) {
        const float4* eb = ws.slab_cur();
        const float4 e0 = eb[lane], e1 = eb[64 + lane];
        y0 = make_float4(act_bwd<P, ACTB>(y0.x, e0.x), act_bwd<P, ACTB>(y0.y, e0.y), act_bwd<P, ACTB>(y0.z, e0.z),
                         act_bwd<P, ACTB>(y0.w, e0.w));
        y1 = make_float4(act_bwd<P, ACTB>(y1.x, e1.x), act_bwd<P, ACTB>(y1.y, e1.y), act_bwd<P, ACTB>(y1.z, e1.z),
                         act_bwd<P, ACTB>(y1.w, e1.w));
      }
      if constexpr (NBO1 > 0) push2<NBO1>(Y, y0, y1);
    } else {
      emb(2 * c - NBO1, y0);
      emb(2 * c + 1 - NBO1, y1);
    }
    ws.flip();
  }
}

__device__ __noinline__ float embed_feature(int f, float x0, float x1, float x2, int nfreq) {
  if (f < 3) return f == 0 ? x0 : (f == 1 ? x1 : x2);
  const int fp = f - 3;
  if (fp >= 6 * nfreq) return 0.0f;
  const int band = fp / 6, m = fp - band * 6, c = m % 3;
  const float xc = c == 0 ? x0 : (c == 1 ? x1 : x2);
  const float v = fmul(xc, (float)(1 << band));
  return m < 3 ? sinf(v) : cosf(v);
}
__device__ __noinline__ void embed_backward(int f, float gf, float x0, float x1, float x2, int nfreq, float& n0,
                                            float& n1, float& n2) {
  float contrib;
  int c;
  if (f < 3) {
    contrib = gf;
    c = f;
  } else {
    const int fp = f - 3;
    if (fp >= 6 * nfreq) return;
    const int band = fp / 6, m = fp - band * 6;
    c = m % 3;
    const float freq = (float)(1 << band);
    const float xc = c == 0 ? x0 : (c == 1 ? x1 : x2);
    const float v = fmul(xc, freq);
    contrib = m < 3 ? fmul(fmul(gf, cosf(v)), freq) : fmul(fmul(gf, -sinf(v)), freq);
  }
  if (c == 0) n0 = fadd(n0, contrib);
  else if (c == 1) n1 = fadd(n1, contrib);
  else n2 = fadd(n2, contrib);
}

__device__ __forceinline__ float wave_sum4(float v) {
  v += __shfl_xor(v, 16);
  v += __shfl_xor(v, 32);
  return v;
}

struct SdfKArgs {
  const char* packed;
  SdfLayout L;
  const float* pts;
  int64_t P;
  float* sdf;
  float* nabla;
  float* feature;
  float4* scratch;
  int nfreq;
  const int* P_dev;
  int P_mult;
  float4* slabs;
  const int* tiles;
  const int* n_tiles;
};

template <int P, bool NABLA>
__global__ __launch_bounds__(kThreads) void sdf_kernel(SdfKArgs a) {
  constexpr int CB = chunk_bytes(18);
  __shared__ __attribute__((aligned(16))) char smem[kRing * CB + (NABLA ? 2 * kSlabChunk : 0)];
  WStream<CB> ws{smem, NABLA ? smem + kRing * CB : nullptr, 0, 0, 0};
  const int lane = threadIdx.x & 63, wave = __builtin_amdgcn_readfirstlane(threadIdx.x >> 6);
  const int j = lane & 15, g = lane >> 4;
  const SdfLayout& L = a.L;
  const char* W = a.packed;
  auto OP = [&](int i) { return W + L.op_off[i]; };
  auto OPB = [&](int i) { return (int)L.op_bytes[i]; };
  const float* w8 = (const float*)(W + L.w8row0_off);
  const float b8 = *(const float*)(W + L.misc_off);
  float4* escr = uniform_ptr(a.scratch + (size_t)(blockIdx.x * kWaves + wave) * (8 * 16 * 64));
  const bool want_feat = a.feature != nullptr;

  ws.start(OP(F0), OPB(F0), OP(F0) + OPB(F0), OPB(F0));

  const int64_t Pn = a.P_dev ? min(a.P, (int64_t)(*a.P_dev) * a.P_mult) : a.P;
  for (int64_t base = (int64_t)blockIdx.x * kPointsPerWG; base < Pn; base += (int64_t)gridDim.x * kPointsPerWG) {
    const bool has_next = base + (int64_t)gridDim.x * kPointsPerWG < Pn;
    const int64_t p = base + wave * kTile + j;
    const bool valid = p < Pn;
    const int64_t pc = valid ? p : Pn - 1;
    const float x0 = a.pts[pc * 3 + 0], x1 = a.pts[pc * 3 + 1], x2 = a.pts[pc * 3 + 2];

    float4 E[4];
#pragma unroll
    for (int b = 0; b < 4; ++b) {
      const int f = 16 * b + 4 * g;
      E[b] = make_float4(embed_feature(f + 0, x0, x1, x2, a.nfreq), embed_feature(f + 1, x0, x1, x2, a.nfreq),
                         embed_feature(f + 2, x0, x1, x2, a.nfreq), embed_feature(f + 3, x0, x1, x2, a.nfreq));
    }
    float4 X[16], Y[16];
    float4* e_l[8];
#pragma unroll
    for (int l = 0; l < 8; ++l) e_l[l] = NABLA ? escr + l * 16 * 64 : nullptr;

    gemm_fwd<P, 0, 4, 16, ACT_SOFTPLUS>(ws, OP(F0), OP(F1), OPB(F1), X, E, Y, e_l[0], nullptr, false, lane);
    gemm_fwd<P, 16, 0, 16, ACT_SOFTPLUS>(ws, OP(F1), OP(F2), OPB(F2), Y, E, X, e_l[1], nullptr, false, lane);
    gemm_fwd<P, 16, 0, 16, ACT_SOFTPLUS>(ws, OP(F2), OP(F3), OPB(F3), X, E, Y, e_l[2], nullptr, false, lane);
    gemm_fwd<P, 16, 0, 14, ACT_SOFTPLUS>(ws, OP(F3), OP(F4), OPB(F4), Y, E, X, e_l[3], nullptr, false, lane);
    gemm_fwd<P, 14, 4, 16, ACT_SOFTPLUS>(ws, OP(F4), OP(F5), OPB(F5), X, E, Y, e_l[4], nullptr, false, lane);
    gemm_fwd<P, 16, 0, 16, ACT_SOFTPLUS>(ws, OP(F5), OP(F6), OPB(F6), Y, E, X, e_l[5], nullptr, false, lane);
    gemm_fwd<P, 16, 0, 16, ACT_SOFTPLUS>(ws, OP(F6), OP(F7), OPB(F7), X, E, Y, e_l[6], nullptr, false, lane);
    {
      const char* n = want_feat ? OP(F8) : (NABLA ? OP(B7) : (has_next ? OP(F0) : nullptr));
      const int nb = want_feat ? OPB(F8) : (NABLA ? OPB(B7) : OPB(F0));
      gemm_fwd<P, 16, 0, 16, ACT_SOFTPLUS>(ws, OP(F7), n, nb, Y, E, X, e_l[7], nullptr, false, lane);
    }
    float part = 0.0f;
#pragma unroll
    for (int b = 0; b < 16; ++b) {
      const float4 w = *(const float4*)(w8 + 16 * b + 4 * g);
      part = fmaf(X[b].x, w.x, part);
      part = fmaf(X[b].y, w.y, part);
      part = fmaf(X[b].z, w.z, part);
      part = fmaf(X[b].w, w.w, part);
    }
    const float sdf = wave_sum4(part) + b8;
    if (valid && g == 0) a.sdf[p] = sdf;
    if (want_feat) {
      const char* n = NABLA ? OP(B7) : (has_next ? OP(F0) : nullptr);
      const int nb = NABLA ? OPB(B7) : OPB(F0);
      gemm_fwd<P, 16, 0, 16, ACT_NONE>(ws, OP(F8), n, nb, X, E, Y, nullptr, a.feature + pc * 256, valid,
                                    lane);
    }
    if constexpr (NABLA) {
#pragma unroll
      for (int b = 0; b < 16; ++b) {
        const float4 w = *(const float4*)(w8 + 16 * b + 4 * g);
        const float4 e = e_l[7][b * 64 + lane];
        X[b] = make_float4(softplus_bwd<P>(w.x, e.x), softplus_bwd<P>(w.y, e.y), softplus_bwd<P>(w.z, e.z),
                           softplus_bwd<P>(w.w, e.w));
      }
      float4* park = e_l[7];
      auto emb_skip = [&](int eb, float4 gv) { park[eb * 64 + lane] = gv; };
      auto emb_first = [&](int eb, float4 gv) { park[(4 + eb) * 64 + lane] = gv; };
      auto noemb = [](int, float4) {};
      ws.slab_now(e_l[6], 0);
      gemm_bwd<P, 16, 16, 0>(ws, OP(B7), OP(B6), OPB(B6), X, Y, e_l[6], e_l[5], lane, noemb);
// ... 574 lines not shown
      sp = fmaf(y[q][1].z, w1.z, sp); sp = fmaf(y[q][1].w, w1.w, sp);
      sdf_part[q] = sp;
      if constexpr (NABLA) {
        pd.v[q] = mul4(w0, s[q][0]);
        pd.v[kNC + q] = mul4(w1, s[q][1]);
      }
      if constexpr (FEAT) {
        mrun[q] = amax8(mrun[q], y[q][0], y[q][1]);
        split8a(y[q][0], y[q][1], sc[q], oh[q][c], ol[q][c]);
      }
    }
    if constexpr (NABLA)
      if (st == 7) pend_chunk(pd, g7, 2 * c, lane, kFeatNT);
  }
};

template <int NMAIN, class WS>
struct BwdEpi4 {
  f16x8 (&oh)[kNC][12];
  f16x8 (&ol)[kNC][12];
  const float (&sc)[kNC];
  WS& ws;
  float4* park;
  int park_blk;
  float (&mrun)[kNC];
  Pend4& pd;
  int lane;
  int plane;
  float4 y[kNC][2];
  __device__ __forceinline__ void operator()(int c, const Z4& zz, int st) {
    if (2 * c < NMAIN) {
      const int q = st >> 2, k = st & 3;
      if (q >= kNC) return;
      if (k < 2) {
        const uint4 sw = *(const uint4*)((const char*)ws.slab_read() + ((kNC * k + q) * 64 + lane) * 16);
        y[q][k] = unpack24_mul(sw.x, sw.y, sw.z, zz.z[q][k]);
      } else if (k == 2) {
        mrun[q] = amax8(mrun[q], y[q][0], y[q][1]);
      } else {
        split8a(y[q][0], y[q][1], sc[q], oh[q][c], ol[q][c]);
        if (q == kNC - 1) ws.slab_consumed();
      }
    } else if (st == 7) {
#pragma unroll
      for (int q = 0; q < kNC; ++q) {
        pd.v[q] = zz.z[q][0];
        pd.v[kNC + q] = zz.z[q][1];
      }
      pend_chunk(pd, park, park_blk + 2 * c - NMAIN, plane, false);
    }
  }
};

struct NoPre4 {
  __device__ __forceinline__ int operator()(int) const { return 0; }
};

template <bool NABLA, bool FEAT, int STAGE_>
__global__ __attribute__((amdgpu_flat_work_group_size(STAGE_ == 3 ? 256 : kT4, STAGE_ == 3 ? 256 : kT4),
                          amdgpu_waves_per_eu(kWPE, kWPE)))
void sdf4_kernel(SdfKArgs a) {
  constexpr int STAGE = STAGE_ == 3 ? 0 : (STAGE_ == 4 ? 2 : STAGE_);
  constexpr bool COMPACT = STAGE_ == 4;
  constexpr int NW = STAGE_ == 3 ? 4 : kW4;
  static_assert(STAGE_ != 3 || (!NABLA && !FEAT), "narrow tiles: forward-only launches");
  static_assert(STAGE == 0 || (NABLA && !FEAT), "deferred nablas: no feature");
  constexpr int PPW = 16 * kNC * NW;
  constexpr int CB = chunk_bytes(18);
  constexpr int C16 = chunk_bytes(16), C4 = chunk_bytes(4), C14 = chunk_bytes(14), C18 = chunk_bytes(18);
  static_assert((size_t)kW4 * kNC * kSlabColBytes <= kScratchPerWG, "per-workgroup slab scratch");
  constexpr bool SLABS = NABLA && STAGE != 1;
  constexpr int RING = SLABS ? 3 : kFwdRing;
  __shared__ __attribute__((aligned(16))) char smem[RING * CB + (SLABS ? kSlabRing * kSlab4 : 0)];
  static_assert(RING * CB + (SLABS ? kSlabRing * kSlab4 : 0) <= 160 * 1024, "LDS budget");
  WStream4<CB, RING, NW> ws{smem, SLABS ? smem + RING * CB : nullptr, 0, 0, 0, 0};
  const int lane = threadIdx.x & 63, wave = __builtin_amdgcn_readfirstlane(threadIdx.x >> 6);
  const int j = lane & 15, g = lane >> 4;
  const char* W = a.packed;
  auto OP = [&](int i) {
    const char* w = W;
    asm volatile("" : "+s"(w));
    return w + sdf_op_off(i);
  };
  const float b8 = *(const float*)(W + a.L.misc_off);
  float4* escr = uniform_ptr((float4*)((char*)a.scratch + (size_t)(blockIdx.x * kW4 + wave) * (kNC * kSlabColBytes)));
  auto slab = [&](int l) {
    char* e = (char*)escr;
    asm volatile("" : "+s"(e));
    return (float4*)(e + l * kNC * kSlab24Layer);
  };

#ifdef NR_EXP_STAMPS
  if ((threadIdx.x & 63) == 0)
    for (int i = 0; i < kStampPh; ++i) stamp_lds()[wave * kStampPh + i] = 0;
#endif
  if constexpr (STAGE == 2) ws.template start<C16, C16>(OP(B7), OP(B7) + C16);
  else if constexpr (RING == 4) ws.template start<C4, C4, C4>(OP(F0), OP(F0) + C4, OP(F0) + 2 * C4);
  else ws.template start<C4, C4>(OP(F0), OP(F0) + C4);
  Pend4 pd{};
  NoPre4 nopre;
  const float kSpSlack = 0.0070f;

  const int64_t Pn = COMPACT      ? ((int64_t)(*a.n_tiles) + 15) / 16 * 16
                     : STAGE == 2 ? (int64_t)(*a.n_tiles) * kPointsPerWG / kW4
                                  : (a.P_dev ? min(a.P, (int64_t)(*a.P_dev) * a.P_mult) : a.P);
  for (int64_t base = (int64_t)blockIdx.x * PPW; base < Pn; base += (int64_t)gridDim.x * PPW) {
    const bool has_next = base + (int64_t)gridDim.x * PPW < Pn;
    int64_t p0 = base + wave * 16 * kNC;
    int plane = lane;
    uint32_t soff = 0;
    int64_t pl = 0;
    bool listed = true;
    if constexpr (COMPACT) {
      const int64_t n = *a.n_tiles;
      const int64_t w0 = p0 < n ? p0 : n - 16;
      const int e = a.tiles[w0 + j];
      const int e0 = __builtin_amdgcn_readfirstlane(a.tiles[w0]);
      listed = p0 < n && e >= 0;
      pl = e >= 0 ? e : e0;
      const uint32_t rt = (uint32_t)((pl >> 4) - (e0 >> 4)), js = (uint32_t)(pl & 15);
      plane = (int)(rt * (uint32_t)(kSlabColBytes / 16) + js + 16u * (uint32_t)g);
      soff = rt * (uint32_t)kSlabColBytes + (js + 16u * (uint32_t)g) * (uint32_t)kSlabVB;
      escr = uniform_ptr((float4*)((char*)a.slabs + (size_t)(e0 >> 4) * kSlabColBytes));
    } else if constexpr (STAGE == 2) {
      const int64_t ti = min(p0 / 16, (int64_t)(*a.n_tiles) - 1);
      const int64_t tile = a.tiles[ti];
      escr = uniform_ptr((float4*)((char*)a.slabs + (size_t)tile * kSlabColBytes));
      p0 = p0 / 16 < (int64_t)(*a.n_tiles) ? tile * 16 : a.P;
    } else if constexpr (STAGE == 1) {
      escr = uniform_ptr((float4*)((char*)a.slabs + (size_t)(p0 / 16) * kSlabColBytes));
    }
    const int64_t Pv = STAGE == 2 ? a.P : Pn;
    int64_t pq[kNC];
    bool valid[kNC];
    float xs[kNC][3];
#pragma unroll
    for (int q = 0; q < kNC; ++q) {
      const int64_t p = p0 + 16 * q + j;
      if constexpr (COMPACT) {
        valid[q] = listed;
        pq[q] = pl;
      } else {
        valid[q] = p < Pv;
        pq[q] = valid[q] ? p : Pv - 1;
      }
      xs[q][0] = a.pts[pq[q] * 3 + 0];
      xs[q][1] = a.pts[pq[q] * 3 + 1];
      xs[q][2] = a.pts[pq[q] * 3 + 2];
    }
    float4 E[kNC][4];
    float mE[kNC], xinv[kNC];
    f16x8 Uh[kNC][12], Ul[kNC][12], Vh[kNC][12], Vl[kNC][12];
    float mrun[kNC], m_in[kNC];
    auto next_scales = [&](int kb, float extra, const float (&floor_max)[kNC], float (&sc)[kNC]) {
      const float4 v = ws.buf()[2 * kb * 64 + 8];
#pragma unroll
      for (int q = 0; q < kNC; ++q) sc[q] = bound_scale(fmaxf(fmaf(v.y, m_in[q], v.z) + extra, floor_max[q]));
    };
    auto finish = [&](const float (&sc)[kNC], float mscale = 1.0f) {
#pragma unroll
      for (int q = 0; q < kNC; ++q) {
        m_in[q] = max4_groups(mrun[q]) * mscale;
        mrun[q] = 0.0f;
        xinv[q] = 1.0f / sc[q];
      }
    };
// ... 21 lines not shown
    if constexpr (NABLA) {
      const uint32_t l = opaque_lane(lane);
#pragma unroll
      for (int q = 0; q < kNC; ++q)
#pragma unroll
        for (int b = 0; b < 4; ++b) {
          const uint32_t off = (((12 + b) * kNC + q) * 64 + l) * 16u;
          const f32x4 d = tof(E[q][b]);
          asm volatile("global_store_dwordx4 %0, %1, %2\n\ts_nop 1" : : "v"(off), "v"(d), "s"(epark) : "memory");
        }
    }
#pragma unroll
    for (int q = 0; q < kNC; ++q) {
      mrun[q] = 0.0f;
      m_in[q] = mE[q];
    }
    auto fwd_epi = [&](f16x8(&oh)[kNC][12], f16x8(&ol)[kNC][12], const float (&sc)[kNC], float4* sl) {
      return FwdEpi4<NABLA>{oh, ol, sc, sl, mrun, pd, lane};
    };

    {
      float sc[kNC];
      next_scales(4, kSpSlack, zero2, sc);
      op4<4, 16, C16, false, true>(ws, OP(F0), OP(F1), Uh, Ul, xinv, pd, nopre, fwd_epi(Vh, Vl, sc, slab(0)), lane);
      finish(sc, kC);
    }
    {
      float sc[kNC];
      next_scales(16, kSpSlack, zero2, sc);
      op4<16, 16, C16, false, true>(ws, OP(F1), OP(F2), Vh, Vl, xinv, pd, nopre, fwd_epi(Uh, Ul, sc, slab(1)), lane);
      finish(sc, kC);
    }
    {
      float sc[kNC];
      next_scales(16, kSpSlack, zero2, sc);
      op4<16, 16, C16, false, true>(ws, OP(F2), OP(F3), Uh, Ul, xinv, pd, nopre, fwd_epi(Vh, Vl, sc, slab(2)), lane);
      finish(sc, kC);
    }
    {
      float sc[kNC];
      next_scales(16, kSpSlack, mE, sc);
      op4<16, 14, C18, false, true>(ws, OP(F3), OP(F4), Vh, Vl, xinv, pd, nopre, fwd_epi(Uh, Ul, sc, slab(3)), lane);
      if constexpr (NABLA) {
        asm volatile("s_waitcnt vmcnt(0)" ::: "memory");
#pragma unroll
        for (int q = 0; q < kNC; ++q)
#pragma unroll
          for (int b = 0; b < 4; ++b) E[q][b] = fromf(*((const gf4*)epark + ((12 + b) * kNC + q) * 64 + lane));
      }
#pragma unroll
      for (int q = 0; q < kNC; ++q) {
        split8a(E[q][0], E[q][1], sc[q], Uh[q][7], Ul[q][7]);
        split8a(E[q][2], E[q][3], sc[q], Uh[q][8], Ul[q][8]);
        mrun[q] = fmaxf(mrun[q], mE[q] * (1.0f / kC));
      }
      finish(sc, kC);
    }
    {
      float sc[kNC];
      next_scales(18, kSpSlack, zero2, sc);
      op4<18, 16, C16, false, true>(ws, OP(F4), OP(F5), Uh, Ul, xinv, pd, nopre, fwd_epi(Vh, Vl, sc, slab(4)), lane);
      finish(sc, kC);
    }
    {
      float sc[kNC];
      next_scales(16, kSpSlack, zero2, sc);
      op4<16, 16, C16, false, true>(ws, OP(F5), OP(F6), Vh, Vl, xinv, pd, nopre, fwd_epi(Uh, Ul, sc, slab(5)), lane);
      finish(sc, kC);
    }
    {
      float sc[kNC];
      next_scales(16, kSpSlack, zero2, sc);
      op4<16, 16, C16, false, true>(ws, OP(F6), OP(F7), Uh, Ul, xinv, pd, nopre, fwd_epi(Vh, Vl, sc, slab(6)), lane);
      finish(sc, kC);
    }
    float sdf_part[kNC];
#pragma unroll
    for (int q = 0; q < kNC; ++q) sdf_part[q] = 0.0f;
    {
      float sc[kNC];
      next_scales(16, kSpSlack, zero2, sc);
      F7Epi4<NABLA, FEAT> epi{Uh, Ul, sc, slab(7), mrun, sdf_part, pd, lane};
      constexpr int NXT = ((NABLA && STAGE == 0) || FEAT) ? C16 : C4;
      const char* n = FEAT ? OP(F8) : ((NABLA && STAGE == 0) ? OP(B7) : (has_next ? OP(F0) : nullptr));
      op4<16, 16, NXT, true, false>(ws, OP(F7), n, Vh, Vl, xinv, pd, nopre, epi, lane);
      finish(sc);
    }
#pragma unroll
    for (int q = 0; q < kNC; ++q) {
      const float sdf = wave_sum4(sdf_part[q]) + b8;
      if (valid[q] && g == 0) a.sdf[p0 + 16 * q + j] = sdf;
    }
    if constexpr (FEAT) {
      const int64_t pf = p0 < Pn ? p0 : Pn - 1;
      float4* fb = uniform_ptr((float4*)(a.feature + pf * 256));
      uint32_t frow[kNC];
#pragma unroll
      for (int q = 0; q < kNC; ++q) frow[q] = (uint32_t)(pq[q] - pf);
      auto epi = [&](int c, const Z4& zz, int st) {
        if (st != 7) return;
#pragma unroll
        for (int q = 0; q < kNC; ++q) {
          pd.v[2 * q] = zz.z[q][0];
          pd.v[2 * q + 1] = zz.z[q][1];
          const uint32_t r = opaque_lane(frow[q] * 64 + g);
          pd.o[2 * q] = r + (2 * c) * 4;
          pd.o[2 * q + 1] = r + (2 * c + 1) * 4;
        }
        pd.put(fb, 2 * kNC, kFeatNT);
      };
      constexpr int NXT = NABLA ? C16 : C4;
      const char* n = NABLA ? OP(B7) : (has_next ? OP(F0) : nullptr);
      op4<16, 16, NXT, false, false>(ws, OP(F8), n, Uh, Ul, xinv, pd, nopre, epi, lane);
    }
    }
    if constexpr (NABLA && STAGE == 1) {
      pd.flush();
    }
    if constexpr (NABLA && STAGE != 1) {
      pd.flush();
      asm volatile("s_waitcnt vmcnt(0)" ::: "memory");
      float4* g7 = slab(7);
#pragma unroll
      for (int q = 0; q < kNC; ++q) {
        float4 G[16];
#pragma unroll
        for (int b = 0; b < 16; ++b) G[b] = fromf(*((const gf4*)g7 + (kNC * b + q) * 64 + (COMPACT ? plane : lane)));
        float m = 0.0f;
#pragma unroll
        for (int b = 0; b < 16; b += 2) m = amax8(m, G[b], G[b + 1]);
        m_in[q] = max4_groups(m);
        mrun[q] = 0.0f;
        const float sc = bound_scale(m_in[q]);
#pragma unroll
        for (int s = 0; s < 8; ++s) split8a(G[2 * s], G[2 * s + 1], sc, Uh[q][s], Ul[q][s]);
        xinv[q] = 1.0f / sc;
      }
      float4* park = slab(7);
      if constexpr (COMPACT) ws.stage_slab(slab(6), 0, soff);
      else ws.stage_slab(slab(6), 0);
      auto bwd = [&](auto kb_tag, auto nbo_tag, auto nmain_tag, auto nxt_tag, int opi, const char* nxt,
                     f16x8(&ih)[kNC][12], f16x8(&il)[kNC][12], f16x8(&oh)[kNC][12], f16x8(&ol)[kNC][12], int lcur,
                     int park_blk, int lnext) {
        constexpr int KBo = decltype(kb_tag)::value, NBOo = decltype(nbo_tag)::value;
        constexpr int NMAIN = decltype(nmain_tag)::value, NXC = decltype(nxt_tag)::value;
        float sc[kNC];
        next_scales(KBo, 0.0f, zero2, sc);
        auto pre = [&](int c) -> int {
          if constexpr (COMPACT) {
            if (2 * (c + 1) < NMAIN) return ws.stage_slab(slab(lcur), c + 1, soff);
            if (c + 1 == NBOo / 2 && lnext >= 0) return ws.stage_slab(slab(lnext), 0, soff);
          } else {
            if (2 * (c + 1) < NMAIN) return ws.stage_slab(slab(lcur), c + 1);
            if (c + 1 == NBOo / 2 && lnext >= 0) return ws.stage_slab(slab(lnext), 0);
          }
          return 0;
        };
        BwdEpi4<NMAIN, decltype(ws)> epi{oh, ol, sc, ws, park, park_blk, mrun, pd, lane, COMPACT ? plane : lane};
        op4<KBo, NBOo, NXC, false, false>(ws, OP(opi), nxt, ih, il, xinv, pd, pre, epi, lane);
        finish(sc);
      };
      using I0 = std::integral_constant<int, 0>;
      using I4 = std::integral_constant<int, 4>;
      using I14 = std::integral_constant<int, 14>;
      using I16 = std::integral_constant<int, 16>;
      using I18 = std::integral_constant<int, 18>;
      using IC16 = std::integral_constant<int, C16>;
      using IC14 = std::integral_constant<int, C14>;
      using IC4 = std::integral_constant<int, C4>;
      bwd(I16{}, I16{}, I16{}, IC16{}, B7, OP(B6), Uh, Ul, Vh, Vl, 6, 0, 5);
      bwd(I16{}, I16{}, I16{}, IC16{}, B6, OP(B5), Vh, Vl, Uh, Ul, 5, 0, 4);
      bwd(I16{}, I16{}, I16{}, IC16{}, B5, OP(B4), Uh, Ul, Vh, Vl, 4, 0, 3);
      bwd(I16{}, I18{}, I14{}, IC14{}, B4, OP(B3), Vh, Vl, Uh, Ul, 3, 0, 2);
      bwd(I14{}, I16{}, I16{}, IC16{}, B3, OP(B2), Uh, Ul, Vh, Vl, 2, 0, 1);
      bwd(I16{}, I16{}, I16{}, IC16{}, B2, OP(B1), Vh, Vl, Uh, Ul, 1, 0, 0);
      bwd(I16{}, I16{}, I16{}, IC16{}, B1, OP(B0), Uh, Ul, Vh, Vl, 0, 0, -1);
      if constexpr (STAGE == 2) bwd(I16{}, I4{}, I0{}, IC16{}, B0, has_next ? OP(B7) : nullptr, Vh, Vl, Uh, Ul, 0, 4, -1);
      else bwd(I16{}, I4{}, I0{}, IC4{}, B0, has_next ? OP(F0) : nullptr, Vh, Vl, Uh, Ul, 0, 4, -1);
      pd.flush();
      asm volatile("s_waitcnt vmcnt(0)" ::: "memory");
#pragma unroll
      for (int q = 0; q < kNC; ++q) {
        float n0 = 0.f, n1 = 0.f, n2 = 0.f;
#pragma unroll
        for (int b = 0; b < 4; ++b) {
          const float4 u = fromf(*((const gf4*)park + (kNC * b + q) * 64 + (COMPACT ? plane : lane)));
          const float4 v = fromf(*((const gf4*)park + (kNC * (4 + b) + q) * 64 + (COMPACT ? plane : lane)));
          const int f = 16 * b + 4 * g;
          embed_backward(f + 0, fadd(v.x, u.x), xs[q][0], xs[q][1], xs[q][2], a.nfreq, n0, n1, n2);
          embed_backward(f + 1, fadd(v.y, u.y), xs[q][0], xs[q][1], xs[q][2], a.nfreq, n0, n1, n2);
          embed_backward(f + 2, fadd(v.z, u.z), xs[q][0], xs[q][1], xs[q][2], a.nfreq, n0, n1, n2);
          embed_backward(f + 3, fadd(v.w, u.w), xs[q][0], xs[q][1], xs[q][2], a.nfreq, n0, n1, n2);
        }
        n0 = wave_sum4(n0);
        n1 = wave_sum4(n1);
        n2 = wave_sum4(n2);
// ... 35 lines not shown
  ws.start(OP(S0), OPB(S0), OP(S0) + OPB(S0), OPB(S0));

  const int64_t Pn = a.P_dev ? min(a.P, (int64_t)(*a.P_dev) * a.P_mult) : a.P;
  for (int64_t base = (int64_t)blockIdx.x * kPointsPerWG; base < Pn; base += (int64_t)gridDim.x * kPointsPerWG) {
    const bool has_next = base + (int64_t)gridDim.x * kPointsPerWG < Pn;
    const int64_t p = base + wave * kTile + j;
    const bool valid = p < Pn;
    const int64_t pc = valid ? p : Pn - 1;
    const float x0 = a.pts[pc * 3 + 0], x1 = a.pts[pc * 3 + 1], x2 = a.pts[pc * 3 + 2];
    float4 E[4];
    E[0] = g == 0 ? make_float4(x0, x1, x2, 0.f) : make_float4(0.f, 0.f, 0.f, 0.f);
#pragma unroll
    for (int b = 1; b < 4; ++b) E[b] = make_float4(0.f, 0.f, 0.f, 0.f);
    float4 X[16], Y[16];
    float4* e_l[5];
#pragma unroll
    for (int l = 0; l < 5; ++l) e_l[l] = NABLA ? escr + l * 16 * 64 : nullptr;

    gemm_fwd<P, 0, 4, 16, ACT_SINE>(ws, OP(S0), OP(S1), OPB(S1), X, E, Y, e_l[0], nullptr, false, lane);
    gemm_fwd<P, 16, 0, 16, ACT_SINE>(ws, OP(S1), OP(S2), OPB(S2), Y, E, X, e_l[1], nullptr, false, lane);
    gemm_fwd<P, 16, 0, 16, ACT_SINE>(ws, OP(S2), OP(S3), OPB(S3), X, E, Y, e_l[2], nullptr, false, lane);
    gemm_fwd<P, 16, 0, 16, ACT_SINE>(ws, OP(S3), OP(S4), OPB(S4), Y, E, X, e_l[3], nullptr, false, lane);
    {
      const char* n = want_feat ? OP(SF) : (NABLA ? OP(SB4) : (has_next ? OP(S0) : nullptr));
      const int nb = want_feat ? OPB(SF) : (NABLA ? OPB(SB4) : OPB(S0));
      gemm_fwd<P, 16, 0, 16, ACT_SINE>(ws, OP(S4), n, nb, X, E, Y, e_l[4], nullptr, false, lane);
    }
    float part = 0.0f;
#pragma unroll
    for (int b = 0; b < 16; ++b) {
      const float4 w = *(const float4*)(wl + 16 * b + 4 * g);
      part = fmaf(Y[b].x, w.x, part);
      part = fmaf(Y[b].y, w.y, part);
      part = fmaf(Y[b].z, w.z, part);
      part = fmaf(Y[b].w, w.w, part);
    }
    const float sdf = wave_sum4(part) + bl;
    if (valid && g == 0) a.sdf[p] = sdf;
    if (want_feat) {
      const char* n = NABLA ? OP(SB4) : (has_next ? OP(S0) : nullptr);
      const int nb = NABLA ? OPB(SB4) : OPB(S0);
      gemm_fwd<P, 16, 0, 16, ACT_NONE>(ws, OP(SF), n, nb, Y, E, X, nullptr, a.feature + pc * 256, valid, lane);
    }
    if constexpr (NABLA) {
#pragma unroll
      for (int b = 0; b < 16; ++b) {
        const float4 w = *(const float4*)(wl + 16 * b + 4 * g);
        const float4 e = e_l[4][b * 64 + lane];
        X[b] = make_float4(sine_bwd(w.x, e.x), sine_bwd(w.y, e.y), sine_bwd(w.z, e.z), sine_bwd(w.w, e.w));
      }
      auto noemb = [](int, float4) {};
      auto coords = [&](int eb, float4 gv) {
        if (eb == 0 && g == 0 && valid) {
          a.nabla[p * 3 + 0] = gv.x;
          a.nabla[p * 3 + 1] = gv.y;
          a.nabla[p * 3 + 2] = gv.z;
        }
      };
      ws.slab_now(e_l[3], 0);
      gemm_bwd<P, 16, 16, 0, ACT_SINE>(ws, OP(SB4), OP(SB3), OPB(SB3), X, Y, e_l[3], e_l[2], lane, noemb);
      gemm_bwd<P, 16, 16, 0, ACT_SINE>(ws, OP(SB3), OP(SB2), OPB(SB2), Y, X, e_l[2], e_l[1], lane, noemb);
      gemm_bwd<P, 16, 16, 0, ACT_SINE>(ws, OP(SB2), OP(SB1), OPB(SB1), X, Y, e_l[1], e_l[0], lane, noemb);
      gemm_bwd<P, 16, 16, 0, ACT_SINE>(ws, OP(SB1), OP(SB0), OPB(SB0), Y, X, e_l[0], nullptr, lane, noemb);
      gemm_bwd<P, 16, 0, 4, ACT_SINE>(ws, OP(SB0), has_next ? OP(S0) : nullptr, OPB(S0), X, Y, nullptr, nullptr,
                                      lane, coords);
    }
  }
  wait_vmcnt(0);
}

struct RadKArgs {
  const char* packed;
  RadLayout L;
  const float* x;
  const float* vdir;
  int64_t vdiv;
  int64_t vmod;
  const float* normals;
  const float* feature;
  int64_t P;
  float* rgb;
  int nfreq_view;
  const int* P_dev;
};

__device__ __forceinline__ float rad_small_feature(int f, const float (&x)[3], const float (&v)[3],
                                                   const float (&n)[3], int nfreq_view, bool view) {
  if (f < 3) return x[f];
  if (!view) return 0.0f;
  f -= 3;
  const int nv = nfreq_view < 0 ? 3 : 3 + 6 * nfreq_view;
  if (f < nv) return embed_feature(f, v[0], v[1], v[2], nfreq_view < 0 ? 0 : nfreq_view);
  f -= nv;
  if (f < 3) return n[f];
  return 0.0f;
}

template <int P, int KBS, int ACT, int D>
__global__ __launch_bounds__(kThreads) void radiance_kernel(RadKArgs a) {
  static_assert(D == 4 || D == 5, "radiance net depth");
  constexpr int CB = chunk_bytes(16 + KBS);
  __shared__ __attribute__((aligned(16))) char smem[kRing * CB];
  WStream<CB> ws{smem, nullptr, 0, 0, 0};
  const int lane = threadIdx.x & 63, wave = __builtin_amdgcn_readfirstlane(threadIdx.x >> 6);
  const int j = lane & 15, g = lane >> 4;
  const RadLayout& L = a.L;
  const char* W = a.packed;
  auto OP = [&](int i) { return W + L.op_off[i]; };
  auto OPB = [&](int i) { return (int)L.op_bytes[i]; };
  const float* head = (const float*)(W + L.head_off);
  const bool view = L.view != 0;

  ws.start(OP(0), OPB(0), OP(0) + OPB(0), OPB(0));
  const int64_t Pn = a.P_dev ? min(a.P, (int64_t)*a.P_dev) : a.P;
  for (int64_t base = (int64_t)blockIdx.x * kPointsPerWG; base < Pn; base += (int64_t)gridDim.x * kPointsPerWG) {
    const bool has_next = base + (int64_t)gridDim.x * kPointsPerWG < Pn;
    const int64_t p = base + wave * kTile + j;
    const bool valid = p < Pn;
    const int64_t pc = valid ? p : Pn - 1;
    float xs[3], vs[3] = {0.f, 0.f, 0.f}, ns[3] = {0.f, 0.f, 0.f};
    const int64_t pv = (pc / a.vdiv) % a.vmod;
#pragma unroll
    for (int c = 0; c < 3; ++c) {
      xs[c] = a.x[pc * 3 + c];
      if (view) {
        vs[c] = a.vdir[pv * 3 + c];
        ns[c] = a.normals[pc * 3 + c];
      }
    }
    float4 S[4];
#pragma unroll
    for (int b = 0; b < 4; ++b) {
      const int f = 16 * b + 4 * g;
      S[b] = b < KBS ? make_float4(rad_small_feature(f, xs, vs, ns, a.nfreq_view, view),
                                   rad_small_feature(f + 1, xs, vs, ns, a.nfreq_view, view),
                                   rad_small_feature(f + 2, xs, vs, ns, a.nfreq_view, view),
                                   rad_small_feature(f + 3, xs, vs, ns, a.nfreq_view, view))
                     : make_float4(0, 0, 0, 0);
    }
    float4 X[16], Y[16];
#pragma unroll
    for (int b = 0; b < 16; ++b) X[b] = *(const float4*)(a.feature + pc * 256 + 16 * b + 4 * g);

    gemm_fwd<P, 16, KBS, 16, ACT>(ws, OP(0), OP(1), OPB(1), X, S, Y, nullptr, nullptr, false, lane);
    gemm_fwd<P, 16, 0, 16, ACT>(ws, OP(1), OP(2), OPB(2), Y, S, X, nullptr, nullptr, false, lane);
    gemm_fwd<P, 16, 0, 16, ACT>(ws, OP(2), OP(3), OPB(3), X, S, Y, nullptr, nullptr, false, lane);
    if constexpr (D == 4) {
      gemm_fwd<P, 16, 0, 16, ACT>(ws, OP(3), has_next ? OP(0) : nullptr, OPB(0), Y, S, X, nullptr, nullptr, false,
                                  lane);
    } else {
      gemm_fwd<P, 16, 0, 16, ACT>(ws, OP(3), OP(4), OPB(4), Y, S, X, nullptr, nullptr, false, lane);
      gemm_fwd<P, 16, 0, 16, ACT>(ws, OP(4), has_next ? OP(0) : nullptr, OPB(0), X, S, Y, nullptr, nullptr, false,
                                  lane);
    }
    const float4(&H)[16] = D == 4 ? X : Y;
    float r[3];
#pragma unroll
    for (int o = 0; o < 3; ++o) {
      float part = 0.f;
#pragma unroll
      for (int b = 0; b < 16; ++b) {
        const float4 w = *(const float4*)(head + o * 256 + 16 * b + 4 * g);
        part = fmaf(H[b].x, w.x, part);
        part = fmaf(H[b].y, w.y, part);
        part = fmaf(H[b].z, w.z, part);
        part = fmaf(H[b].w, w.w, part);
// ... 65 lines not shown
    store(0, Y);
    gemm_fwd<NR_PREC_FP32, 16, 0, 16, ACT_RELU>(ws, OP(1), OP(2), OPB(2), Y, S, X, nullptr, nullptr, false, lane);
    store(1, X);
    gemm_fwd<NR_PREC_FP32, 16, 0, 16, ACT_RELU>(ws, OP(2), OP(3), OPB(3), X, S, Y, nullptr, nullptr, false, lane);
    store(2, Y);
    gemm_fwd<NR_PREC_FP32, 16, 0, 16, ACT_RELU>(ws, OP(3), has_next ? OP(0) : nullptr, OPB(0), Y, S, X, nullptr,
                                                nullptr, false, lane);
    store(3, X);
    float r[3];
#pragma unroll
    for (int o = 0; o < 3; ++o) {
      float part = 0.f;
#pragma unroll
      for (int b = 0; b < 16; ++b) {
        const float4 w = *(const float4*)(head + o * 256 + 16 * b + 4 * g);
        part = fmaf(X[b].x, w.x, part);
        part = fmaf(X[b].y, w.y, part);
        part = fmaf(X[b].z, w.z, part);
        part = fmaf(X[b].w, w.w, part);
      }
      r[o] = sigmoidf_ref(wave_sum4(part) + head[3 * 256 + o]);
    }
    if (valid && g == 0) {
      a.rgb[p * 3 + 0] = r[0];
      a.rgb[p * 3 + 1] = r[1];
      a.rgb[p * 3 + 2] = r[2];
    }
  }
  wait_vmcnt(0);
}

struct ReluEpi4 {
  f16x8 (&oh)[kNC][12];
  f16x8 (&ol)[kNC][12];
  const float (&sc)[kNC];
  float (&mrun)[kNC];
  float4 y[kNC][2];
  __device__ __forceinline__ void operator()(int c, const Z4& zz, int st) {
    const int q = st >> 2, k = st & 3;
    if (q >= kNC) return;
    if (k < 2) {
      const float4 z = zz.z[q][k];
      y[q][k] = make_float4(fmaxf(z.x, 0.0f), fmaxf(z.y, 0.0f), fmaxf(z.z, 0.0f), fmaxf(z.w, 0.0f));
    } else if (k == 2) {
      mrun[q] = amax8(mrun[q], y[q][0], y[q][1]);
    } else {
      split8a(y[q][0], y[q][1], sc[q], oh[q][c], ol[q][c]);
    }
  }
};

struct HeadEpi4 {
  const float* head;
  float (&part)[kNC][3];
  int g;
  float4 y[kNC][2];
  __device__ __forceinline__ void operator()(int c, const Z4& zz, int st) {
    const int q = st >> 2, k = st & 3;
    if (q >= kNC) return;
    if (k < 2) {
      const float4 z = zz.z[q][k];
      y[q][k] = make_float4(fmaxf(z.x, 0.0f), fmaxf(z.y, 0.0f), fmaxf(z.z, 0.0f), fmaxf(z.w, 0.0f));
    } else {
#pragma unroll
      for (int o = 0; o < 3; ++o) {
        if ((o == 0) != (k == 2)) continue;
        float p = part[q][o];
        const uint32_t lo = opaque_lane(4 * g);
#pragma unroll
        for (int b = 0; b < 2; ++b) {
          const float4 w = *(const float4*)(head + lo + o * 256 + 16 * (2 * c + b));
          p = fmaf(y[q][b].x, w.x, p);
          p = fmaf(y[q][b].y, w.y, p);
          p = fmaf(y[q][b].z, w.z, p);
          p = fmaf(y[q][b].w, w.w, p);
        }
        asm volatile("" : "+v"(p));
        part[q][o] = p;
      }
    }
  }
};

template <int KBS>
__global__ __attribute__((amdgpu_flat_work_group_size(kT4, kT4), amdgpu_waves_per_eu(kWPE, kWPE)))
void rad4_kernel(RadKArgs a) {
  constexpr int K0 = 16 + KBS;
  constexpr int C0 = chunk_bytes(K0), C16 = chunk_bytes(16);
  __shared__ __attribute__((aligned(16))) char smem[kRing * C0 + (3 * 256 + 4) * 4];
  static_assert(kRing * C0 + (3 * 256 + 4) * 4 <= 160 * 1024, "LDS budget");
  WStream4<C0> ws{smem, nullptr, 0, 0, 0};
  float* head = (float*)(smem + kRing * C0);
  const int lane = threadIdx.x & 63, wave = __builtin_amdgcn_readfirstlane(threadIdx.x >> 6);
  const int j = lane & 15, g = lane >> 4;
  const RadLayout& L = a.L;
  const char* W = a.packed;
  auto OP = [&](int i) {
    const char* w = W;
    asm volatile("" : "+s"(w));
    return w + L.op_off[i];
  };
  const bool view = L.view != 0;
  {
    const float* hsrc = (const float*)(W + L.head_off);
    for (int i = threadIdx.x; i < 3 * 256 + 4; i += kT4) head[i] = hsrc[i];
  }
  ws.template start<C0, C0>(OP(0), OP(0) + C0);
  Pend4 pd{};
  NoPre4 nopre;
  const int64_t Pn = a.P_dev ? min(a.P, (int64_t)*a.P_dev) : a.P;
  for (int64_t base = (int64_t)blockIdx.x * kPointsPerWG; base < Pn; base += (int64_t)gridDim.x * kPointsPerWG) {
    const bool has_next = base + (int64_t)gridDim.x * kPointsPerWG < Pn;
    const int64_t p0 = base + wave * 16 * kNC;
    f16x8 Uh[kNC][12], Ul[kNC][12], Vh[kNC][12], Vl[kNC][12];
    float m_in[kNC], xinv[kNC], mrun[kNC];
    bool valid[kNC];
#pragma unroll
    for (int q = 0; q < kNC; ++q) {
      const int64_t p = p0 + 16 * q + j;
      valid[q] = p < Pn;
      const int64_t pc = valid[q] ? p : Pn - 1;
      const int64_t pv = (pc / a.vdiv) % a.vmod;
      float xs[3], vs[3] = {0.f, 0.f, 0.f}, ns[3] = {0.f, 0.f, 0.f};
#pragma unroll
      for (int c = 0; c < 3; ++c) {
        xs[c] = a.x[pc * 3 + c];
        if (view) {
          vs[c] = a.vdir[pv * 3 + c];
          ns[c] = a.normals[pc * 3 + c];
        }
      }
      float4 X[16 + KBS];
      const int gq = (int)opaque_lane(g);
#pragma unroll
      for (int b = 0; b < KBS; ++b) {
        const int f = 16 * b + 4 * gq;
        X[16 + b] = make_float4(rad_small_feature(f, xs, vs, ns, a.nfreq_view, view),
                                rad_small_feature(f + 1, xs, vs, ns, a.nfreq_view, view),
                                rad_small_feature(f + 2, xs, vs, ns, a.nfreq_view, view),
                                rad_small_feature(f + 3, xs, vs, ns, a.nfreq_view, view));
      }
#pragma unroll
      for (int b = 0; b < 16; ++b) X[b] = *(const float4*)(a.feature + pc * 256 + 16 * b + 4 * g);
      float m = 0.0f;
#pragma unroll
      for (int b = 0; b < 16 + KBS; b += 2) m = amax8(m, X[b], X[b + 1]);
      m_in[q] = max4_groups(m);
      const float s = bound_scale(m_in[q]);
#pragma unroll
      for (int k = 0; k < K0 / 2; ++k) split8a(X[2 * k], X[2 * k + 1], s, Uh[q][k], Ul[q][k]);
      xinv[q] = 1.0f / s;
      mrun[q] = 0.0f;
    }
    auto next_scales = [&](int kb, float (&sc)[kNC]) {
      const float4 v = ws.buf()[2 * kb * 64 + 8];
#pragma unroll
      for (int q = 0; q < kNC; ++q) sc[q] = bound_scale(fmaf(v.y, m_in[q], v.z));
    };
    auto finish = [&](const float (&sc)[kNC]) {
#pragma unroll
      for (int q = 0; q < kNC; ++q) {
        m_in[q] = max4_groups(mrun[q]);
        mrun[q] = 0.0f;
        xinv[q] = 1.0f / sc[q];
      }
    };
    {
      float sc[kNC];
      next_scales(K0, sc);
      op4<K0, 16, C16, false, false>(ws, OP(0), OP(1), Uh, Ul, xinv, pd, nopre, ReluEpi4{Vh, Vl, sc, mrun}, lane);
      finish(sc);
    }
    {
      float sc[kNC];
      next_scales(16, sc);
      op4<16, 16, C16, false, false>(ws, OP(1), OP(2), Vh, Vl, xinv, pd, nopre, ReluEpi4{Uh, Ul, sc, mrun}, lane);
      finish(sc);
    }
    {
      float sc[kNC];
      next_scales(16, sc);
      op4<16, 16, C16, false, false>(ws, OP(2), OP(3), Uh, Ul, xinv, pd, nopre, ReluEpi4{Vh, Vl, sc, mrun}, lane);
      finish(sc);
    }
    float part[kNC][3];
#pragma unroll
    for (int q = 0; q < kNC; ++q) part[q][0] = part[q][1] = part[q][2] = 0.0f;
    op4<16, 16, C0, false, false>(ws, OP(3), has_next ? OP(0) : nullptr, Vh, Vl, xinv, pd, nopre,
                                  HeadEpi4{head, part, g}, lane);
#pragma unroll
    for (int q = 0; q < kNC; ++q) {
      float r[3];
#pragma unroll
      for (int o = 0; o < 3; ++o) r[o] = sigmoidf_ref(wave_sum4(part[q][o]) + head[3 * 256 + o]);
      if (valid[q] && g == 0) {
        const int64_t p = p0 + 16 * q + j;
        a.rgb[p * 3 + 0] = r[0];
        a.rgb[p * 3 + 1] = r[1];
        a.rgb[p * 3 + 2] = r[2];
      }
    }
  }
  pd.flush();
  wait_vmcnt(0);
}

struct NerfKArgs {
  const char* packed;
  NerfLayout L;
  const float* x4;
  const float* vdir;
  int64_t vdiv;
  int64_t vmod;
  int64_t P;
  float* sigma;
  float* rgb;
  const int* P_dev;
};

__device__ __noinline__ float nerf_embed4(int f, float x0, float x1, float x2, float x3) {
  auto comp = [&](int c) { return c == 0 ? x0 : (c == 1 ? x1 : (c == 2 ? x2 : x3)); };
  if (f < 4) return comp(f);
  const int fp = f - 4;
  if (fp >= 80) return 0.0f;
  const int band = fp >> 3, m = fp & 7;
  const float v = fmul(comp(m & 3), (float)(1 << band));
  return m < 4 ? sinf(v) : cosf(v);
}

template <int P>
__global__ __launch_bounds__(kThreads) void nerf_kernel(NerfKArgs a) {
  constexpr int CB = chunk_bytes(22);
  __shared__ __attribute__((aligned(16))) char smem[kRing * CB];
  WStream<CB> ws{smem, nullptr, 0, 0, 0};
  const int lane = threadIdx.x & 63, wave = __builtin_amdgcn_readfirstlane(threadIdx.x >> 6);
  const int j = lane & 15, g = lane >> 4;
  const NerfLayout& L = a.L;
  const char* W = a.packed;
  auto OP = [&](int i) { return W + L.op_off[i]; };
  auto OPB = [&](int i) { return (int)L.op_bytes[i]; };
  const float* wa = (const float*)(W + L.alpha_off);
  const float* wr = (const float*)(W + L.rgb_off);

  ws.start(OP(N0), OPB(N0), OP(N0) + OPB(N0), OPB(N0));
  const int64_t Pn = a.P_dev ? min(a.P, (int64_t)*a.P_dev) : a.P;
  for (int64_t base = (int64_t)blockIdx.x * kPointsPerWG; base < Pn; base += (int64_t)gridDim.x * kPointsPerWG) {
    const bool has_next = base + (int64_t)gridDim.x * kPointsPerWG < Pn;
    const int64_t p = base + wave * kTile + j;
    const bool valid = p < Pn;
    const int64_t pc = valid ? p : Pn - 1;
    const float4 xin = *(const float4*)(a.x4 + pc * 4);
    const int64_t pv = (pc / a.vdiv) % a.vmod;
    const float v0 = a.vdir[pv * 3 + 0], v1 = a.vdir[pv * 3 + 1], v2 = a.vdir[pv * 3 + 2];
// ... 1069 lines not shown
  for (int off = 32; off > 0; off >>= 1) {
    best = fmaxf(best, __shfl_xor(best, off));
    bb = fmaxf(bb, __shfl_xor(bb, off));
    m = fmaxf(m, __shfl_xor(m, off));
  }
  if (lane == 0) {
    red[0][wave] = m;
    red[1][wave] = best;
    red[2][wave] = bb;
  }
  __syncthreads();
  if (threadIdx.x == 0) {
    float a = 0.0f, b = 0.0f, c = 0.0f;
    for (int w = 0; w < 4; ++w) {
      a = fmaxf(a, red[0][w]);
      b = fmaxf(b, red[1][w]);
      c = fmaxf(c, red[2][w]);
    }
    if (op.prec == NR_PREC_F16X3) *op.wmax = a;
    if (op.bound) {
      op.bound[0] = b;
      op.bound[1] = c;
    }
  }
}

__global__ void pack_vec_kernel(const float* __restrict__ src, int off, int nvalid, int n, float* __restrict__ dst) {
  const int e = blockIdx.x * blockDim.x + threadIdx.x;
  if (e >= n) return;
  dst[e] = e < nvalid ? src[off + e] : 0.0f;
}

int launch_pack_ops(const PackOp* ops, char* const* dst, int nops, hipStream_t stream) {
  for (int b0 = 0; b0 < nops; b0 += kPackBatch) {
    const int nb = std::min(kPackBatch, nops - b0);
    PackBatch pb{};
    int64_t nmax = 0;
    for (int i = 0; i < nb; ++i) {
      const PackOp& op = ops[b0 + i];
      NR_REQUIRE(op.prec != NR_PREC_F16X3 || op.wmax, NR_ERR_ARG, "pack: f16x3 needs a max-|W| word");
      const int KB = op.in[0].nblk + op.in[1].nblk;
      const int NBO = op.out[0].nblk + op.out[1].nblk;
      pb.op[i] = op;
      pb.dst[i] = (uint32_t*)dst[b0 + i];
      pb.n[i] = (int64_t)(NBO / 2) * (2 * KB + 1) * 256;
      nmax = std::max(nmax, pb.n[i]);
    }
    int gmax = 1;
    for (int i = 0; i < nb; ++i)
      gmax = std::max(gmax, ((pb.op[i].out[0].nblk + pb.op[i].out[1].nblk) * 16 + kPackRowsPerWG - 1) / kPackRowsPerWG);
    NR_REQUIRE(gmax <= 32, NR_ERR_UNSUPPORTED, "pack: more than 512 output rows in one op");
    hipLaunchKernelGGL(pack_rows_kernel, dim3(gmax, nb), dim3(1024), 0, stream, pb);
    NR_HIP_CHECK(hipGetLastError());
    hipLaunchKernelGGL(pack_final_kernel, dim3(nb), dim3(256), 0, stream, pb);
    NR_HIP_CHECK(hipGetLastError());
    hipLaunchKernelGGL(pack_ops_kernel, dim3((unsigned)((nmax + 255) / 256), nb), dim3(256), 0, stream, pb);
    NR_HIP_CHECK(hipGetLastError());
  }
  return NR_OK;
}

int launch_pack_op(const PackOp& op, char* dst, hipStream_t stream) { return launch_pack_ops(&op, &dst, 1, stream); }

int launch_pack_vec(const float* src, int off, int nvalid, int n, char* dst, hipStream_t stream) {
  hipLaunchKernelGGL(pack_vec_kernel, dim3((n + 255) / 256), dim3(256), 0, stream, src, off, nvalid, n, (float*)dst);
  NR_HIP_CHECK(hipGetLastError());
  return NR_OK;
}

static int cu_count() {
  int dev = 0, cus = 256;
  if (hipGetDevice(&dev) == hipSuccess) (void)hipDeviceGetAttribute(&cus, hipDeviceAttributeMultiprocessorCount, dev);
  return cus;
}

static int grid_for(int64_t P, int ppw = kPointsPerWG) {
  const int cus = cu_count();
  const int64_t need = (P + ppw - 1) / ppw;
  return (int)(need < cus ? (need > 0 ? need : 1) : cus);
}

int launch_sdf(const SdfLayout& L, const void* packed, const float* pts, int64_t P, float* sdf, float* nabla,
               float* feature, int nfreq, void* ws, size_t ws_bytes, hipStream_t stream, const int* P_dev,
               int P_mult) {
  if (P <= 0) return NR_OK;
  const int grid = grid_for(P);
  SdfKArgs a{(const char*)packed, L, pts, P, sdf, nabla, feature, (float4*)ws, nfreq, P_dev, P_mult, nullptr, nullptr,
             nullptr};
  ProfScope prof(nabla ? (feature ? "sdf_nabla_feat" : "sdf_nabla") : (feature ? "sdf_feat" : "sdf_fwd"), (double)P,
                 stream, P_dev, P_mult);
  if (L.siren) {
    if (nabla) {
      const size_t need = (size_t)grid * kScratchPerWG;
      NR_REQUIRE(ws && ws_bytes >= need, NR_ERR_WORKSPACE, "sdf nabla workspace too small");
      if (L.prec == NR_PREC_F16X3)
        hipLaunchKernelGGL((siren_sdf_kernel<NR_PREC_F16X3, true>), dim3(grid), dim3(kThreads), 0, stream, a);
      else hipLaunchKernelGGL((siren_sdf_kernel<NR_PREC_FP32, true>), dim3(grid), dim3(kThreads), 0, stream, a);
    } else {
      if (L.prec == NR_PREC_F16X3)
        hipLaunchKernelGGL((siren_sdf_kernel<NR_PREC_F16X3, false>), dim3(grid), dim3(kThreads), 0, stream, a);
      else hipLaunchKernelGGL((siren_sdf_kernel<NR_PREC_FP32, false>), dim3(grid), dim3(kThreads), 0, stream, a);
    }
    NR_HIP_CHECK(hipGetLastError());
    return NR_OK;
  }
  if (nabla) {
    const size_t need = (size_t)grid * kScratchPerWG;
    NR_REQUIRE(ws && ws_bytes >= need, NR_ERR_WORKSPACE, "sdf nabla workspace too small");
    if (L.prec == NR_PREC_F16X3) {
      if (feature) hipLaunchKernelGGL((sdf4_kernel<true, true, 0>), dim3(grid), dim3(kT4), 0, stream, a);
      else hipLaunchKernelGGL((sdf4_kernel<true, false, 0>), dim3(grid), dim3(kT4), 0, stream, a);
    }
    else hipLaunchKernelGGL((sdf_kernel<NR_PREC_FP32, true>), dim3(grid), dim3(kThreads), 0, stream, a);
  } else {
    if (L.prec == NR_PREC_F16X3) {
      if (feature) hipLaunchKernelGGL((sdf4_kernel<false, true, 0>), dim3(grid), dim3(kT4), 0, stream, a);
      else if (P <= (int64_t)64 * cu_count())
        hipLaunchKernelGGL((sdf4_kernel<false, false, 3>), dim3(grid_for(P, 64)), dim3(256), 0, stream, a);
      else hipLaunchKernelGGL((sdf4_kernel<false, false, 0>), dim3(grid), dim3(kT4), 0, stream, a);
    }
    else hipLaunchKernelGGL((sdf_kernel<NR_PREC_FP32, false>), dim3(grid), dim3(kThreads), 0, stream, a);
  }
  NR_HIP_CHECK(hipGetLastError());
  return NR_OK;
}

int launch_sdf_deferred(const SdfLayout& L, const void* packed, const float* pts, int64_t P, float* sdf, float* nabla,
                        int nfreq, float4* slabs, const int* tiles, const int* n_tiles, int stage, hipStream_t stream) {
  if (P <= 0) return NR_OK;
  NR_REQUIRE(L.prec == NR_PREC_F16X3 && !L.siren, NR_ERR_UNSUPPORTED, "deferred nablas: f16x3 softplus nets");
  SdfKArgs a{(const char*)packed, L, pts, P, sdf, nabla, nullptr, nullptr, nfreq, nullptr, 0, slabs, tiles, n_tiles};
  if (stage == 1) {
    ProfScope prof("sdf_nabla_fwd", (double)P, stream);
    hipLaunchKernelGGL((sdf4_kernel<true, false, 1>), dim3(grid_for(P)), dim3(kT4), 0, stream, a);
  } else if (stage == 2) {
    ProfScope prof("sdf_nabla_bwd", (double)P, stream, n_tiles, 16);
    hipLaunchKernelGGL((sdf4_kernel<true, false, 2>), dim3(grid_for(P)), dim3(kT4), 0, stream, a);
  } else {
    NR_REQUIRE(stage == 4, NR_ERR_ARG, "deferred nablas: bad stage");
    ProfScope prof("sdf_nabla_bwd", (double)P, stream, n_tiles, 1);
    hipLaunchKernelGGL((sdf4_kernel<true, false, 4>), dim3(grid_for(P)), dim3(kT4), 0, stream, a);
  }
  NR_HIP_CHECK(hipGetLastError());
  return NR_OK;
}

int launch_nerf(const NerfLayout& L, const void* packed, const float* x4, const float* vdir, int64_t vdiv,
                int64_t vmod, int64_t P, float* sigma, float* rgb, hipStream_t stream, const int* P_dev) {
  if (P <= 0) return NR_OK;
  const int grid = grid_for(P);
  NerfKArgs a{(const char*)packed, L, x4, vdir, vdiv, vmod, P, sigma, rgb, P_dev};
  ProfScope prof("nerf", (double)P, stream, P_dev, 1);
  if (L.prec == NR_PREC_F16X3) hipLaunchKernelGGL(nerf4_kernel, dim3(grid), dim3(kT4), 0, stream, a);
  else hipLaunchKernelGGL((nerf_kernel<NR_PREC_FP32>), dim3(grid), dim3(kThreads), 0, stream, a);
  NR_HIP_CHECK(hipGetLastError());
  return NR_OK;
}

int launch_nerf_train32_fwd(const NerfLayout& L, const void* packed, const float* xe, const float* ve, int64_t P,
                            float* const* h, float* feat, float* hv, float* sigma, float* rgb, hipStream_t stream) {
  if (P <= 0) return NR_OK;
  NR_REQUIRE(L.prec == NR_PREC_FP32, NR_ERR_ARG, "nerf train forward: needs the fp32 render pack");
  NerfTrainFwdArgs a{};
  a.packed = (const char*)packed;
  a.L = L;
  a.xe = xe;
  a.ve = ve;
  a.P = P;
  for (int i = 0; i < 8; ++i) a.h[i] = h[i];
  a.feat = feat;
  a.hv = hv;
  a.sigma = sigma;
  a.rgb = rgb;
  ProfScope prof("nerf_train32_fwd", (double)P, stream);
  hipLaunchKernelGGL(nerf_train32_fwd_kernel, dim3(grid_for(P)), dim3(kThreads), 0, stream, a);
  NR_HIP_CHECK(hipGetLastError());
  return NR_OK;
}

int launch_nerf_train32_bwd(const NerfBwdLayout& B, const void* packed, const float* rgb, const float* hv,
                            const float* const* h, const float* g_rgb, const float* g_sigma, int64_t P, float* g3,
                            float* ghv, float* g_feat, float* const* gz, hipStream_t stream,
                            bool f16x3) {
  if (P <= 0) return NR_OK;
  NerfTrainBwdArgs a{};
  a.packed = (const char*)packed;
  a.B = B;
  a.rgb = rgb;
  a.hv = hv;
  for (int i = 0; i < 8; ++i) a.h[i] = h[i];
  a.g_rgb = g_rgb;
  a.g_sigma = g_sigma;
  a.P = P;
  a.g3 = g3;
  a.ghv = ghv;
  a.g_feat = g_feat;
  for (int i = 0; i < 8; ++i) a.gz[i] = gz[i];
  ProfScope prof("nerf_train32_bwd", (double)P, stream);
  if (f16x3) hipLaunchKernelGGL(nerf_train32_bwd_kernel<NR_PREC_F16X3>, dim3(grid_for(P)), dim3(kThreads), 0, stream, a);
  else hipLaunchKernelGGL(nerf_train32_bwd_kernel<NR_PREC_FP32>, dim3(grid_for(P)), dim3(kThreads), 0, stream, a);
  NR_HIP_CHECK(hipGetLastError());
  return NR_OK;
}

int launch_radiance_train32(const RadLayout& L, const void* packed, const float* feat, const float* small,
                            int64_t ld_small, int n_small, int64_t P, float* const* h, float* rgb, hipStream_t stream) {
  if (P <= 0) return NR_OK;
  if (L.prec != NR_PREC_FP32 || L.siren || L.D != 4 || (L.kbs != 2 && L.kbs != 4)) {
    set_error("nr_radiance_train_fwd32: needs the fp32 pack of a ReLU D=4 radiance net");
    return NR_ERR_UNSUPPORTED;
  }
  RadTrainArgs a{(const char*)packed, L, feat, small, ld_small, n_small, P, {h[0], h[1], h[2], h[3]}, rgb};
  ProfScope prof("radiance_train32", (double)P, stream);
  if (L.kbs == 2) hipLaunchKernelGGL((radiance_train32_kernel<2>), dim3(grid_for(P)), dim3(kThreads), 0, stream, a);
  else hipLaunchKernelGGL((radiance_train32_kernel<4>), dim3(grid_for(P)), dim3(kThreads), 0, stream, a);
  NR_HIP_CHECK(hipGetLastError());
  return NR_OK;
}

int launch_radiance(const RadLayout& L, const void* packed, const float* x, const float* vdir, int64_t vdiv,
                    int64_t vmod, const float* normals, const float* feature, int64_t P, float* rgb, int nfreq_view,
                    hipStream_t stream, const int* P_dev) {
  if (P <= 0) return NR_OK;
  const int grid = grid_for(P);
  RadKArgs a{(const char*)packed, L, x, vdir, vdiv, vmod, normals, feature, P, rgb, nfreq_view, P_dev};
  ProfScope prof("radiance", (double)P, stream, P_dev, 1);
  const bool h3 = L.prec == NR_PREC_F16X3;
#define NR_RAD_LAUNCH(KBS, ACT, D)                                                                            \
  do {                                                                                                        \
    if (h3) hipLaunchKernelGGL((radiance_kernel<NR_PREC_F16X3, KBS, ACT, D>), dim3(grid), dim3(kThreads), 0, \
                               stream, a);                                                                    \
    else hipLaunchKernelGGL((radiance_kernel<NR_PREC_FP32, KBS, ACT, D>), dim3(grid), dim3(kThreads), 0,     \
                            stream, a);                                                                       \
  } while (0)
  if (L.kbs != 2 && L.kbs != 4) {
    set_error("radiance: unsupported small-input block count");
    return NR_ERR_UNSUPPORTED;
  }
  if (h3 && !L.siren && L.D == 4) {
    if (L.kbs == 2) hipLaunchKernelGGL((rad4_kernel<2>), dim3(grid), dim3(kT4), 0, stream, a);
    else hipLaunchKernelGGL((rad4_kernel<4>), dim3(grid), dim3(kT4), 0, stream, a);
  } else if (!L.siren && L.D == 4) {
    if (L.kbs == 2) NR_RAD_LAUNCH(2, ACT_RELU, 4); else NR_RAD_LAUNCH(4, ACT_RELU, 4);
  } else if (!L.siren && L.D == 5) {
    if (L.kbs == 2) NR_RAD_LAUNCH(2, ACT_RELU, 5); else NR_RAD_LAUNCH(4, ACT_RELU, 5);
  } else if (L.D == 4) {
    if (L.kbs == 2) NR_RAD_LAUNCH(2, ACT_SINE, 4); else NR_RAD_LAUNCH(4, ACT_SINE, 4);
  } else {
    if (L.kbs == 2) NR_RAD_LAUNCH(2, ACT_SINE, 5); else NR_RAD_LAUNCH(4, ACT_SINE, 5);
  }
#undef NR_RAD_LAUNCH
  NR_HIP_CHECK(hipGetLastError());
  return NR_OK;
}

}

#ifdef NR_EXP_STAMPS
extern "C" int nr_exp_stamps(unsigned long long* out, int n) {
  return hipMemcpyFromSymbol(out, HIP_SYMBOL(nr::g_nr_stamps), sizeof(unsigned long long) * (size_t)n) == hipSuccess
             ? nr::kW4 * nr::kStampPh
             : -1;
}
#endif
```

### neurecon_amd/frameworks/neus.py

```python
import copy
import ctypes
import math
from collections import OrderedDict

import numpy as np
import torch
import torch.nn as nn
import torch.nn.functional as F

from .. import _lib as L
from ..base import ImplicitSurface, NeRF, RadianceNet, _no_training, check_view_dirs, wants_graph
from .. import rend_util


class NeuS(nn.Module):

    def __init__(self, variance_init=0.05, speed_factor=1.0, input_ch=3, W_geo_feat=-1, use_outside_nerf=False,
                 obj_bounding_radius=1.0, surface_cfg=dict(), radiance_cfg=dict()):
        super().__init__()
        self.ln_s = nn.Parameter(data=torch.Tensor([-np.log(variance_init) / speed_factor]), requires_grad=True)
        self.speed_factor = speed_factor
        self.implicit_surface = ImplicitSurface(W_geo_feat=W_geo_feat, input_ch=input_ch,
                                                obj_bounding_size=obj_bounding_radius, **surface_cfg)
        if W_geo_feat < 0:
            W_geo_feat = self.implicit_surface.W
        self.radiance_net = RadianceNet(W_geo_feat=W_geo_feat, **radiance_cfg)
        if use_outside_nerf:
            self.nerf_outside = NeRF(input_ch=4, multires=10, multires_view=4, use_view_dirs=True)

    def forward_radiance(self, x, view_dirs):
        _, nablas, geometry_feature = self.implicit_surface.forward_with_nablas(x)
        return self.radiance_net.forward(x, view_dirs, nablas, geometry_feature)

    def forward_s(self):
        return torch.exp(self.ln_s * self.speed_factor)

    def forward(self, x, view_dirs):
        sdf, nablas, geometry_feature = self.implicit_surface.forward_with_nablas(x)
        radiances = self.radiance_net.forward(x, view_dirs, nablas, geometry_feature)
        return radiances, sdf, nablas


_TABLES = {}


def _linspace_table(n, device):
    key = (n, str(device))
    t = _TABLES.get(key)
    if t is None:
        t = torch.linspace(0, 1, n).float().to(device)
        _TABLES[key] = t
    return t


def _neus_uniforms(B, N, batched, rayschunk, direct, n_iters, n_up, N_importance, N_outside, dev):
    pre = [B] if batched else []
    rd = 1 + len(pre) if not direct else len(pre)
    ups, outs = [], []
    for r0 in range(0, N, rayschunk):
        nc = min(rayschunk, N - r0)
        if direct:
            ups.append(rend_util.uniform([*pre, nc, N_importance], dev))
        elif n_iters > 0:
            ups.append(torch.stack([rend_util.uniform([*pre, nc, n_up], dev) for _ in range(n_iters)], 0))
        if N_outside > 0:
            outs.append(rend_util.to_device(rend_util.uniform([*pre, nc, N_outside]).float(), dev))
    u = None
    if ups:
        u = torch.cat(ups, rd)
        u = (u.reshape(B * N, N_importance) if direct else u.reshape(n_iters, B * N, n_up)).contiguous()
    t_out = torch.cat(outs, len(pre)).reshape(B * N, N_outside).contiguous() if outs else None
    return u, t_out


def volume_render(rays_o, rays_d, model, obj_bounding_radius=1.0, batched=False, batched_info={},
                  calc_normal=False, use_view_dirs=True, rayschunk=65536, netchunk=1048576, white_bkgd=False,
                  near_bypass=None, far_bypass=None, detailed_output=True, show_progress=False, perturb=False,
                  fixed_s_recp=1 / 64., N_samples=64, N_importance=64, N_outside=0,
                  upsample_algo='official_solution', N_nograd_samples=2048, N_upsample_iters=4,
                  skip_zero_alpha=True, defer_sample_nablas=True, max_workspace_gb=None, **dummy_kwargs):
    L.require_gpu(rays_o, 'rays_o')
    if wants_graph(model):
        return _train_render(rays_o, rays_d, model, obj_bounding_radius=obj_bounding_radius, batched=batched,
                             calc_normal=calc_normal, use_view_dirs=use_view_dirs, rayschunk=rayschunk,
                             white_bkgd=white_bkgd, near_bypass=near_bypass, far_bypass=far_bypass,
                             detailed_output=detailed_output, perturb=perturb, fixed_s_recp=fixed_s_recp,
                             N_samples=N_samples, N_importance=N_importance, N_outside=N_outside,
                             upsample_algo=upsample_algo, N_nograd_samples=N_nograd_samples,
                             N_upsample_iters=N_upsample_iters)
    if upsample_algo not in L.UPSAMPLE:
        raise NotImplementedError(upsample_algo)
    direct = upsample_algo != 'official_solution'
    check_view_dirs(model, use_view_dirs)
    dev = rays_o.device
    if batched:
        B = rays_d.shape[0]
        prefix = [B, -1]
    else:
        prefix = [-1]
    ro = rays_o.reshape(-1, 3).float().contiguous()
    rd = rays_d.reshape(-1, 3).float().contiguous()
    n = ro.shape[0]
    if direct:
        n_up = N_importance
        S = N_samples + N_importance
    else:
        n_up = N_importance // N_upsample_iters if N_upsample_iters > 0 else 0
        S = N_samples + N_upsample_iters * n_up
    M = S - 1 + N_outside

    sdf_desc, sdf_packed = model.implicit_surface.nr_packed(dev)
    rad_desc, rad_packed = model.radiance_net.nr_packed(dev)
    s_dev = model.forward_s().detach().float().reshape(-1)[:1].contiguous()
    t_coarse = _linspace_table(N_samples, dev)
    u_fine = _linspace_table(max(n_up, 1), dev)

    rgb = torch.empty(n, 3, device=dev)
    depth = torch.empty(n, device=dev)
    acc = torch.empty(n, device=dev)
    normals = torch.empty(n, 3, device=dev) if calc_normal else None
    det = {}
    if detailed_output:
        det = dict(implicit_nablas=torch.empty(n, S, 3, device=dev), implicit_surface=torch.empty(n, S, device=dev),
                   radiance=torch.empty(n, M, 3, device=dev), alpha=torch.empty(n, M, device=dev),
                   cdf=torch.empty(n, S, device=dev), visibility_weights=torch.empty(n, M, device=dev),
                   d_final=torch.empty(n, M, device=dev))
        if N_outside > 0:
            det['sigma_out'] = torch.empty(n, M, device=dev)
            det['radiance_out'] = torch.empty(n, M, 3, device=dev)
    a = L.NrNeusArgs()
    a.rays_o, a.rays_d, a.n_rays = L.ptr(ro), L.ptr(rd), n
    a.sdf, a.sdf_packed = ctypes.pointer(sdf_desc), L.ptr(sdf_packed)
    a.rad, a.rad_packed = ctypes.pointer(rad_desc), L.ptr(rad_packed)
    a.s, a.s_dev = 0.0, L.ptr(s_dev)
    a.no_mid_skip = 0 if skip_zero_alpha else 1
    a.no_defer = 0 if defer_sample_nablas else 1
    a.max_chunk_rays = int(rayschunk) if rayschunk else 0
    a.max_workspace_bytes = L.workspace_budget_bytes(max_workspace_gb)
    a.obj_bounding_radius = float(obj_bounding_radius)
    a.near_bypass = float('nan') if near_bypass is None else float(near_bypass)
    a.far_bypass = float('nan') if far_bypass is None else float(far_bypass)
    a.N_samples, a.N_importance, a.N_upsample_iters = N_samples, N_importance, N_upsample_iters
    a.calc_normal, a.white_bkgd = int(bool(calc_normal)), int(bool(white_bkgd))
    a.t_coarse, a.u_fine = L.ptr(t_coarse), L.ptr(u_fine)
    a.upsample_algo = L.UPSAMPLE[upsample_algo]
    a.fixed_s = 1. / fixed_s_recp
    if upsample_algo == 'direct_more':
        t_nograd = _linspace_table(N_nograd_samples, dev)
        a.N_nograd_samples, a.t_nograd = N_nograd_samples, L.ptr(t_nograd)
    a.rgb, a.depth, a.acc, a.normals = L.ptr(rgb), L.ptr(depth), L.ptr(acc), L.ptr(normals)
    a.d_final = L.ptr(det.get('d_final'))
    a.sdf_out = L.ptr(det.get('implicit_surface'))
    a.nablas_out = L.ptr(det.get('implicit_nablas'))
    a.radiance_out = L.ptr(det.get('radiance'))
    a.alpha_out = L.ptr(det.get('alpha'))
    a.cdf_out = L.ptr(det.get('cdf'))
    a.weights_out = L.ptr(det.get('visibility_weights'))
    if N_outside > 0:
        if not hasattr(model, 'nerf_outside'):
            raise ValueError('N_outside > 0 needs a model built with use_outside_nerf=True')
        nerf_desc, nerf_packed = model.nerf_outside.nr_packed(dev)
        t_out = _linspace_table(N_outside + 2, dev)
        a.nerf, a.nerf_packed = ctypes.pointer(nerf_desc), L.ptr(nerf_packed)
        a.N_outside, a.t_outside = N_outside, L.ptr(t_out)
        a.sigma_out, a.radiance_bg_out = L.ptr(det.get('sigma_out')), L.ptr(det.get('radiance_out'))
    if perturb:
        B = rays_d.shape[0] if batched else 1
        u_rand, t_out_rand = _neus_uniforms(B, n // B, batched, int(rayschunk), direct, N_upsample_iters, n_up,
                                            N_importance, N_outside, dev)
        a.u_rand, a.t_out_rand = L.ptr(u_rand), L.ptr(t_out_rand)
    lib = L.lib()
    ws_bytes = lib.nr_neus_workspace_bytes(ctypes.byref(a))
    ws = L.workspace(dev, ws_bytes)
    a.workspace, a.workspace_bytes = L.ptr(ws), ws_bytes
    L.check(lib.nr_neus_render(ctypes.byref(a), L.stream_of(dev)))

    ret = OrderedDict([('rgb', rgb.reshape(*prefix, 3)), ('depth_volume', depth.reshape(prefix)),
                       ('mask_volume', acc.reshape(prefix))])
    if calc_normal:
        ret['normals_volume'] = normals.reshape(*prefix, 3)
    if detailed_output:
        ret['implicit_nablas'] = det['implicit_nablas'].reshape(*prefix, S, 3)
        ret['implicit_surface'] = det['implicit_surface'].reshape(*prefix, S)
        ret['radiance'] = det['radiance'].reshape(*prefix, M, 3)
        ret['alpha'] = det['alpha'].reshape(*prefix, M)
        ret['cdf'] = det['cdf'].reshape(*prefix, S)
        ret['visibility_weights'] = det['visibility_weights'].reshape(*prefix, M)
        ret['d_final'] = det['d_final'].reshape(*prefix, M)
        if N_outside > 0:
            ret['sigma_out'] = det['sigma_out'].reshape(*prefix, M)
            ret['radiance_out'] = det['radiance_out'].reshape(*prefix, M, 3)
    return ret['rgb'], ret['depth_volume'], ret


def _sample_depths(ro, rd, model, dev, obj_bounding_radius, batched, B, rayschunk, near_bypass, far_bypass, perturb,
                   fixed_s_recp, N_samples, N_importance, upsample_algo, N_nograd_samples, N_upsample_iters,
                   N_outside=0):
    direct = upsample_algo != 'official_solution'
    n = ro.shape[0]
    n_up = N_importance if direct else (N_importance // N_upsample_iters if N_upsample_iters > 0 else 0)
    S = N_samples + (N_importance if direct else N_upsample_iters * n_up)
    sdf_desc, sdf_packed = model.implicit_surface.nr_packed(dev)
    rad_desc = model.radiance_net.nr_desc()
    d_all = torch.empty(n, S, device=dev)
    a = L.NrNeusArgs()
    a.rays_o, a.rays_d, a.n_rays = L.ptr(ro), L.ptr(rd), n
    a.sdf, a.sdf_packed = ctypes.pointer(sdf_desc), L.ptr(sdf_packed)
    a.rad, a.rad_packed = ctypes.pointer(rad_desc), None
    a.obj_bounding_radius = float(obj_bounding_radius)
    a.near_bypass = float('nan') if near_bypass is None else float(near_bypass)
    a.far_bypass = float('nan') if far_bypass is None else float(far_bypass)
    a.N_samples, a.N_importance, a.N_upsample_iters = N_samples, N_importance, N_upsample_iters
    t_coarse = _linspace_table(N_samples, dev)
    u_fine = _linspace_table(max(n_up, 1), dev)
    a.t_coarse, a.u_fine = L.ptr(t_coarse), L.ptr(u_fine)
    a.upsample_algo = L.UPSAMPLE[upsample_algo]
# ... 226 lines not shown
```

Baseline: 683,200.

## Fold SDF feature output layer into radiance first layer

Precomputes the product of the SDF net's last (feature) layer and the radiance net's first-layer feature weights as a new 256x256 matrix with a fused bias. The SDF kernel then emits that folded pre-activation in place of the feature, and the radiance first layer only multiplies the small positional/view inputs before adding it. This removes a 256-wide K block from the radiance layer-0 GEMM at the cost of an extra cached packed weight buffer. It is on by default for the f16x3 ReLU D=4 configuration and may shift fp16 rounding slightly.

```diff
diff --git a/include/neurecon_hip.h b/include/neurecon_hip.h
--- a/include/neurecon_hip.h
+++ b/include/neurecon_hip.h
@@ -123,6 +123,7 @@
   int no_defer;
   int64_t max_chunk_rays;
   size_t max_workspace_bytes;
+  const void* fold_packed;
 } NrNeusArgs;
 
 #define NR_DEFAULT_WORKSPACE_BYTES ((size_t)4 << 30)
@@ -130,6 +131,13 @@
 
 size_t nr_neus_workspace_bytes(const NrNeusArgs* a);
 int nr_neus_render(const NrNeusArgs* a, void* stream);
+
+size_t nr_neus_fold_packed_bytes(const NrSdfDesc* sdf, const NrRadDesc* rad);
+int nr_neus_fold_pack(const NrSdfDesc* sdf, const NrRadDesc* rad, const float* W8, const float* b8, const float* W0,
+                      const float* b0, void* packed, void* stream);
+int nr_neus_fold_forward(const NrSdfDesc* sdf, const void* sdf_packed, const NrRadDesc* rad, const void* rad_packed,
+                         const void* fold_packed, const float* pts, const float* vdir, int64_t vdir_div,
+                         const float* normals, int64_t P, float* u, float* sdf_out, float* rgb, void* stream);
 
 typedef struct {
   const float* rays_o;
diff --git a/neurecon_amd/_lib.py b/neurecon_amd/_lib.py
--- a/neurecon_amd/_lib.py
+++ b/neurecon_amd/_lib.py
@@ -52,6 +52,7 @@
         ('workspace', _c_p), ('workspace_bytes', _c_sz),
         ('u_rand', _c_p), ('t_out_rand', _c_p), ('s_dev', _c_p), ('sample_only', _c_i), ('d_all_out', _c_p),
         ('no_mid_skip', _c_i), ('no_defer', _c_i), ('max_chunk_rays', _c_i64), ('max_workspace_bytes', _c_sz),
+        ('fold_packed', _c_p),
     ]
 
 
@@ -170,6 +171,11 @@
                                    _c_i64, _c_p, _c_p, _c_p, ctypes.POINTER(_c_p), _c_p]),
     'nr_neus_workspace_bytes': (_c_sz, [ctypes.POINTER(NrNeusArgs)]),
     'nr_neus_render': (_c_i, [ctypes.POINTER(NrNeusArgs), _c_p]),
+    'nr_neus_fold_packed_bytes': (_c_sz, [ctypes.POINTER(NrSdfDesc), ctypes.POINTER(NrRadDesc)]),
+    'nr_neus_fold_pack': (_c_i, [ctypes.POINTER(NrSdfDesc), ctypes.POINTER(NrRadDesc), _c_p, _c_p, _c_p, _c_p, _c_p,
+                                 _c_p]),
+    'nr_neus_fold_forward': (_c_i, [ctypes.POINTER(NrSdfDesc), _c_p, ctypes.POINTER(NrRadDesc), _c_p, _c_p, _c_p, _c_p,
+                                    _c_i64, _c_p, _c_i64, _c_p, _c_p, _c_p, _c_p]),
     'nr_volsdf_workspace_bytes': (_c_sz, [ctypes.POINTER(NrVolsdfArgs)]),
     'nr_volsdf_render': (_c_i, [ctypes.POINTER(NrVolsdfArgs), _c_p]),
     'nr_unisurf_workspace_bytes': (_c_sz, [ctypes.POINTER(NrUnisurfArgs)]),
diff --git a/neurecon_amd/base.py b/neurecon_amd/base.py
--- a/neurecon_amd/base.py
+++ b/neurecon_amd/base.py
@@ -316,6 +316,25 @@
         self._nr_cache = (key, desc, packed, Ws, bs)
         return desc, packed
 
+    def nr_fold_packed(self, implicit_surface, device):
+        sdf_desc, _ = implicit_surface.nr_packed(device)
+        rad_desc, _ = self.nr_packed(device)
+        key = (implicit_surface._nr_cache[0], self._nr_cache[0])
+        cache = self.__dict__.get('_nr_fold_cache')
+        if cache is not None and cache[0] == key:
+            return cache[1]
+        lib = L.lib()
+        nbytes = lib.nr_neus_fold_packed_bytes(ctypes.byref(sdf_desc), ctypes.byref(rad_desc))
+        packed = None
+        if nbytes:
+            sW, sb = implicit_surface._nr_cache[3], implicit_surface._nr_cache[4]
+            rW, rb = self._nr_cache[3], self._nr_cache[4]
+            packed = torch.empty(nbytes, dtype=torch.uint8, device=device)
+            L.check(lib.nr_neus_fold_pack(ctypes.byref(sdf_desc), ctypes.byref(rad_desc), L.ptr(sW[-1]), L.ptr(sb[-1]),
+                                          L.ptr(rW[0]), L.ptr(rb[0]), L.ptr(packed), L.stream_of(device)))
+        self.__dict__['_nr_fold_cache'] = (key, packed)
+        return packed
+
     def forward(self, x, view_dirs, normals, geometry_feature):
         L.require_gpu(x, 'points')
         shape = x.shape[:-1]
diff --git a/neurecon_amd/csrc/nr_capi.hip b/neurecon_amd/csrc/nr_capi.hip
--- a/neurecon_amd/csrc/nr_capi.hip
+++ b/neurecon_amd/csrc/nr_capi.hip
@@ -102,6 +102,29 @@
   off = align256(off + (3 * 256 + 4) * 4);
   L.total = (uint32_t)off;
   return L;
+}
+
+bool fold_applies(const NrSdfDesc& sd, const NrRadDesc& rd) {
+  return sd.precision == NR_PREC_F16X3 && !sd.siren && sd.W_geo_feat == 256 && rd.precision == NR_PREC_F16X3 &&
+         !rd.siren && rd.D == 4 && rd.W_geo_feat == 256;
+}
+
+FoldLayout fold_layout(const RadLayout& RL) {
+  FoldLayout F{};
+  F.kbs = RL.kbs;
+  size_t off = 0;
+  F.f8_off = (uint32_t)off;
+  off += 8 * (size_t)chunk_bytes_host(16);
+  F.r0_off = (uint32_t)off;
+  off += 8 * (size_t)chunk_bytes_host(RL.kbs);
+  F.scale_off = (uint32_t)off;
+  off = align256(off + 2 * 4);
+  F.bound_off = (uint32_t)off;
+  off = align256(off + 2 * 2 * 4);
+  F.u_off = (uint32_t)off;
+  off = align256(off + (256 * 256 + 256) * 4);
+  F.total = (uint32_t)off;
+  return F;
 }
 
 int check_nerf_desc(const NrNerfDesc* d) {
@@ -305,12 +328,19 @@
                                  a.sdf->multires, mlp_ws, mlp_bytes, st)))
     return rc;
   const int64_t Pm = (int64_t)(c.S - 1) * R;
+  const char* f8p = nullptr;
+  const char* r0p = nullptr;
+  if (a.fold_packed) {
+    const FoldLayout FL = fold_layout(RL);
+    f8p = (const char*)a.fold_packed + FL.f8_off;
+    r0p = (const char*)a.fold_packed + FL.r0_off;
+  }
   if (a.radiance_out || a.no_mid_skip) {
     if ((rc = launch_sdf(SL, a.sdf_packed, c.mids, Pm, c.sdf_m, c.nab_m, c.feat_m, a.sdf->multires, mlp_ws, mlp_bytes,
-                         st)))
+                         st, nullptr, 0, f8p)))
       return rc;
     if ((rc = launch_radiance(RL, a.rad_packed, c.mids, c.rd, 1, R, c.nab_m, c.feat_m, Pm, c.rad_m,
-                              a.rad->multires_view, st)))
+                              a.rad->multires_view, st, nullptr, r0p)))
       return rc;
   } else {
     char* wsb = (char*)a.workspace;
@@ -325,10 +355,10 @@
                        slot, midc, vdc);
     NR_HIP_CHECK(hipGetLastError());
     if ((rc = launch_sdf(SL, a.sdf_packed, midc, Pm, c.sdf_m, c.nab_m, c.feat_m, a.sdf->multires, mlp_ws, mlp_bytes,
-                         st, cnt, 1)))
+                         st, cnt, 1, f8p)))
       return rc;
     if ((rc = launch_radiance(RL, a.rad_packed, midc, vdc, 1, INT64_MAX, c.nab_m, c.feat_m, Pm, radc,
-                              a.rad->multires_view, st, cnt)))
+                              a.rad->multires_view, st, cnt, r0p)))
       return rc;
     hipLaunchKernelGGL(neus_mid_scatter, g1, dim3(256), 0, st, slot, radc, Pm, c.rad_m);
     NR_HIP_CHECK(hipGetLastError());
@@ -1106,6 +1136,8 @@
              NR_ERR_ARG, "nr_neus_render: null ray or output pointer");
   NR_REQUIRE(a->sdf_packed && a->rad && (a->rad_packed || a->sample_only) && a->t_coarse, NR_ERR_ARG,
              "nr_neus_render: null argument");
+  NR_REQUIRE(!a->fold_packed || fold_applies(*a->sdf, *a->rad), NR_ERR_ARG,
+             "nr_neus_render: a fold pack needs the f16x3 softplus SDF net and a f16x3 ReLU D=4 radiance net");
   NR_REQUIRE(a->N_samples >= 2, NR_ERR_ARG, "nr_neus_render: N_samples must be >= 2");
   NR_REQUIRE(a->n_rays <= 0 || a->sample_only || !a->calc_normal || a->normals, NR_ERR_ARG,
              "nr_neus_render: calc_normal needs normals output");
@@ -1145,6 +1177,63 @@
     if ((rc = neus_chunk(*a, pl, r0, R, (hipStream_t)stream))) return rc;
   }
   return NR_OK;
+}
+
+static int check_fold(const NrSdfDesc* sd, const NrRadDesc* rd) {
+  int rc = check_sdf_desc(sd);
+  if (rc) return rc;
+  if ((rc = check_rad_desc(rd))) return rc;
+  NR_REQUIRE(fold_applies(*sd, *rd), NR_ERR_UNSUPPORTED,
+             "NeuS fold: needs the f16x3 softplus SDF net and a f16x3 ReLU D=4 radiance net");
+  return NR_OK;
+}
+
+size_t nr_neus_fold_packed_bytes(const NrSdfDesc* sd, const NrRadDesc* rd) {
+  if (!sd || !rd || check_sdf_desc(sd) || check_rad_desc(rd) || !fold_applies(*sd, *rd)) return 0;
+  return fold_layout(rad_layout(*rd)).total;
+}
+
+int nr_neus_fold_pack(const NrSdfDesc* sd, const NrRadDesc* rd, const float* W8, const float* b8, const float* W0,
+                      const float* b0, void* packed, void* stream) {
+  int rc = check_fold(sd, rd);
+  if (rc) return rc;
+  NR_REQUIRE(W8 && b8 && W0 && b0 && packed, NR_ERR_ARG, "nr_neus_fold_pack: null argument");
+  hipStream_t st = (hipStream_t)stream;
+  const RadLayout RL = rad_layout(*rd);
+  const FoldLayout F = fold_layout(RL);
+  char* P = (char*)packed;
+  const int ns = RL.n_small, ld0 = ns + 256;
+  float* U = (float*)(P + F.u_off);
+  float* bu = U + 256 * 256;
+  if ((rc = nr_gemm32(W0 + ns, ld0, W8 + 256, 256, 0, nullptr, U, 256, 256, 256, 256, 0, stream))) return rc;
+  if ((rc = nr_gemm32(b8 + 1, 256, W0 + ns, ld0, 1, b0, bu, 256, 1, 256, 256, 0, stream))) return rc;
+  float* wmax = (float*)(P + F.scale_off);
+  float* bound = (float*)(P + F.bound_off);
+  PackOp ops[2];
+  ops[0] = mkop(U, bu, 256, 256, 0, seg(16, 0, 256), none(), seg(16, 0, 256), none(), 1.0f, NR_PREC_F16X3, wmax);
+  ops[1] = mkop(W0, nullptr, 256, ld0, 0, seg(16, 0, 256), none(), seg(RL.kbs, 0, ns), none(), 1.0f, NR_PREC_F16X3,
+                wmax + 1);
+  char* dst[2] = {P + F.f8_off, P + F.r0_off};
+  for (int i = 0; i < 2; ++i) ops[i].bound = bound + 2 * i;
+  return launch_pack_ops(ops, dst, 2, st);
+}
+
+int nr_neus_fold_forward(const NrSdfDesc* sd, const void* sdf_packed, const NrRadDesc* rd, const void* rad_packed,
+                         const void* fold_packed, const float* pts, const float* vdir, int64_t vdir_div,
+                         const float* normals, int64_t P, float* u, float* sdf_out, float* rgb, void* stream) {
+  int rc = check_fold(sd, rd);
+  if (rc) return rc;
+  NR_REQUIRE(sdf_packed && rad_packed && fold_packed && pts && (rd->no_view_dirs || (vdir && normals)) && u &&
+                 sdf_out && rgb && vdir_div > 0 && P >= 0,
+             NR_ERR_ARG, "nr_neus_fold_forward: bad argument");
+  const RadLayout RL = rad_layout(*rd);
+  const FoldLayout F = fold_layout(RL);
+  const char* fp = (const char*)fold_packed;
+  if ((rc = launch_sdf(sdf_layout(*sd), sdf_packed, pts, P, sdf_out, nullptr, u, sd->multires, nullptr, 0,
+                       (hipStream_t)stream, nullptr, 0, fp + F.f8_off)))
+    return rc;
+  return launch_radiance(RL, rad_packed, pts, vdir, vdir_div, INT64_MAX, normals, u, P, rgb, rd->multires_view,
+                         (hipStream_t)stream, nullptr, fp + F.r0_off);
 }
 
 size_t nr_volsdf_workspace_bytes(const NrVolsdfArgs* a) {
diff --git a/neurecon_amd/csrc/nr_mlp.h b/neurecon_amd/csrc/nr_mlp.h
--- a/neurecon_amd/csrc/nr_mlp.h
+++ b/neurecon_amd/csrc/nr_mlp.h
@@ -110,7 +110,8 @@
 int launch_pack_vec(const float* src, int off, int nvalid, int n, char* dst, hipStream_t stream);
 int launch_sdf(const SdfLayout& L, const void* packed, const float* pts, int64_t P, float* sdf, float* nabla,
                float* feature, int nfreq, void* ws, size_t ws_bytes, hipStream_t stream,
-               const int* P_dev = nullptr, int P_mult = 0);
+               const int* P_dev = nullptr, int P_mult = 0,
+               const void* f8_alt = nullptr);
 int launch_sdf_deferred(const SdfLayout& L, const void* packed, const float* pts, int64_t P, float* sdf, float* nabla,
                         int nfreq, float4* slabs, const int* tiles, const int* n_tiles, int stage, hipStream_t stream);
 int launch_nerf(const NerfLayout& L, const void* packed, const float* x4, const float* vdir, int64_t vdiv,
@@ -118,7 +119,19 @@
                 const int* P_dev = nullptr);
 int launch_radiance(const RadLayout& L, const void* packed, const float* x, const float* vdir, int64_t vdiv,
                     int64_t vmod, const float* normals, const float* feature, int64_t P, float* rgb, int nfreq_view,
-                    hipStream_t stream, const int* P_dev = nullptr);
+                    hipStream_t stream, const int* P_dev = nullptr,
+                    const void* r0_fold = nullptr);
+
+struct FoldLayout {
+  uint32_t f8_off, r0_off;
+  uint32_t scale_off;
+  uint32_t bound_off;
+  uint32_t u_off;
+  uint32_t total;
+  int kbs;
+};
+FoldLayout fold_layout(const RadLayout& RL);
+bool fold_applies(const NrSdfDesc& sd, const NrRadDesc& rd);
 
 int launch_radiance_train32(const RadLayout& L, const void* packed, const float* feat, const float* small,
                             int64_t ld_small, int n_small, int64_t P, float* const* h, float* rgb, hipStream_t stream);
diff --git a/neurecon_amd/csrc/nr_mlp.hip b/neurecon_amd/csrc/nr_mlp.hip
--- a/neurecon_amd/csrc/nr_mlp.hip
+++ b/neurecon_amd/csrc/nr_mlp.hip
@@ -490,6 +490,7 @@
   float4* slabs;
   const int* tiles;
   const int* n_tiles;
+  const char* f8_alt;
 };
 
 template <int P, bool NABLA>
@@ -1230,6 +1231,11 @@
     asm volatile("" : "+s"(w));
     return w + sdf_op_off(i);
   };
+  auto OPF8 = [&]() {
+    const char* w = a.f8_alt;
+    asm volatile("" : "+s"(w));
+    return w ? w : OP(F8);
+  };
   const float b8 = *(const float*)(W + a.L.misc_off);
   float4* escr = uniform_ptr((float4*)((char*)a.scratch + (size_t)(blockIdx.x * kW4 + wave) * (kNC * kSlabColBytes)));
   auto slab = [&](int l) {
@@ -1417,7 +1423,9 @@
       next_scales(16, kSpSlack, zero2, sc);
       F7Epi4<NABLA, FEAT> epi{Uh, Ul, sc, slab(7), mrun, sdf_part, pd, lane};
       constexpr int NXT = ((NABLA && STAGE == 0) || FEAT) ? C16 : C4;
-      const char* n = FEAT ? OP(F8) : ((NABLA && STAGE == 0) ? OP(B7) : (has_next ? OP(F0) : nullptr));
+      const char* n;
+      if constexpr (FEAT) n = OPF8();
+      else n = (NABLA && STAGE == 0) ? OP(B7) : (has_next ? OP(F0) : nullptr);
       op4<16, 16, NXT, true, false>(ws, OP(F7), n, Vh, Vl, xinv, pd, nopre, epi, lane);
       finish(sc);
     }
@@ -1446,7 +1454,7 @@
       };
       constexpr int NXT = NABLA ? C16 : C4;
       const char* n = NABLA ? OP(B7) : (has_next ? OP(F0) : nullptr);
-      op4<16, 16, NXT, false, false>(ws, OP(F8), n, Uh, Ul, xinv, pd, nopre, epi, lane);
+      op4<16, 16, NXT, false, false>(ws, OPF8(), n, Uh, Ul, xinv, pd, nopre, epi, lane);
     }
     }
     if constexpr (NABLA && STAGE == 1) {
@@ -1648,6 +1656,7 @@
   float* rgb;
   int nfreq_view;
   const int* P_dev;
+  const char* r0_fold;
 };
 
 __device__ __forceinline__ float rad_small_feature(int f, const float (&x)[3], const float (&v)[3],
@@ -1879,23 +1888,47 @@
   }
 };
 
-template <int KBS>
+struct FoldEpi4 {
+  f16x8 (&oh)[kNC][12];
+  f16x8 (&ol)[kNC][12];
+  const float (&sc)[kNC];
+  float (&mrun)[kNC];
+  const float4 (&u)[kNC][16];
+  float4 y[kNC][2];
+  __device__ __forceinline__ void operator()(int c, const Z4& zz, int st) {
+    const int q = st >> 2, k = st & 3;
+    if (q >= kNC) return;
+    if (k < 2) {
+      const float4 z = zz.z[q][k], v = u[q][2 * c + k];
+      y[q][k] = make_float4(fmaxf(z.x + v.x, 0.0f), fmaxf(z.y + v.y, 0.0f), fmaxf(z.z + v.z, 0.0f),
+                            fmaxf(z.w + v.w, 0.0f));
+    } else if (k == 2) {
+      mrun[q] = amax8(mrun[q], y[q][0], y[q][1]);
+    } else {
+      split8a(y[q][0], y[q][1], sc[q], oh[q][c], ol[q][c]);
+    }
+  }
+};
+
+template <int KBS, bool FOLD>
 __global__ __attribute__((amdgpu_flat_work_group_size(kT4, kT4), amdgpu_waves_per_eu(kWPE, kWPE)))
 void rad4_kernel(RadKArgs a) {
-  constexpr int K0 = 16 + KBS;
+  constexpr int KF = FOLD ? 0 : 16;
+  constexpr int K0 = KF + KBS;
   constexpr int C0 = chunk_bytes(K0), C16 = chunk_bytes(16);
-  __shared__ __attribute__((aligned(16))) char smem[kRing * C0 + (3 * 256 + 4) * 4];
-  static_assert(kRing * C0 + (3 * 256 + 4) * 4 <= 160 * 1024, "LDS budget");
-  WStream4<C0> ws{smem, nullptr, 0, 0, 0};
-  float* head = (float*)(smem + kRing * C0);
+  constexpr int CM = C0 > C16 ? C0 : C16;
+  __shared__ __attribute__((aligned(16))) char smem[kRing * CM + (3 * 256 + 4) * 4];
+  static_assert(kRing * CM + (3 * 256 + 4) * 4 <= 160 * 1024, "LDS budget");
+  WStream4<CM> ws{smem, nullptr, 0, 0, 0};
+  float* head = (float*)(smem + kRing * CM);
   const int lane = threadIdx.x & 63, wave = __builtin_amdgcn_readfirstlane(threadIdx.x >> 6);
   const int j = lane & 15, g = lane >> 4;
   const RadLayout& L = a.L;
   const char* W = a.packed;
   auto OP = [&](int i) {
-    const char* w = W;
+    const char* w = FOLD && i == 0 ? a.r0_fold : W;
     asm volatile("" : "+s"(w));
-    return w + L.op_off[i];
+    return FOLD && i == 0 ? w : w + L.op_off[i];
   };
   const bool view = L.view != 0;
   {
@@ -1911,6 +1944,8 @@
     const int64_t p0 = base + wave * 16 * kNC;
     f16x8 Uh[kNC][12], Ul[kNC][12], Vh[kNC][12], Vl[kNC][12];
     float m_in[kNC], xinv[kNC], mrun[kNC];
+    float4 ufold[kNC][FOLD ? 16 : 1];
+    float umax[kNC];
     bool valid[kNC];
 #pragma unroll
     for (int q = 0; q < kNC; ++q) {
@@ -1927,21 +1962,31 @@
           ns[c] = a.normals[pc * 3 + c];
         }
       }
-      float4 X[16 + KBS];
+      float4 X[K0];
       const int gq = (int)opaque_lane(g);
 #pragma unroll
       for (int b = 0; b < KBS; ++b) {
         const int f = 16 * b + 4 * gq;
-        X[16 + b] = make_float4(rad_small_feature(f, xs, vs, ns, a.nfreq_view, view),
+        X[KF + b] = make_float4(rad_small_feature(f, xs, vs, ns, a.nfreq_view, view),
                                 rad_small_feature(f + 1, xs, vs, ns, a.nfreq_view, view),
                                 rad_small_feature(f + 2, xs, vs, ns, a.nfreq_view, view),
                                 rad_small_feature(f + 3, xs, vs, ns, a.nfreq_view, view));
       }
-#pragma unroll
-      for (int b = 0; b < 16; ++b) X[b] = *(const float4*)(a.feature + pc * 256 + 16 * b + 4 * g);
+      if constexpr (FOLD) {
+#pragma unroll
+        for (int b = 0; b < 16; ++b) ufold[q][b] = *(const float4*)(a.feature + pc * 256 + 16 * b + 4 * g);
+        float mu = 0.0f;
+#pragma unroll
+        for (int b = 0; b < 16; b += 2) mu = amax8(mu, ufold[q][b], ufold[q][b + 1]);
+        umax[q] = max4_groups(mu);
+      } else {
+#pragma unroll
+        for (int b = 0; b < 16; ++b) X[b] = *(const float4*)(a.feature + pc * 256 + 16 * b + 4 * g);
+        umax[q] = 0.0f;
+      }
       float m = 0.0f;
 #pragma unroll
-      for (int b = 0; b < 16 + KBS; b += 2) m = amax8(m, X[b], X[b + 1]);
+      for (int b = 0; b < K0; b += 2) m = amax8(m, X[b], X[b + 1]);
       m_in[q] = max4_groups(m);
       const float s = bound_scale(m_in[q]);
 #pragma unroll
@@ -1964,8 +2009,16 @@
     };
     {
       float sc[kNC];
-      next_scales(K0, sc);
-      op4<K0, 16, C16, false, false>(ws, OP(0), OP(1), Uh, Ul, xinv, pd, nopre, ReluEpi4{Vh, Vl, sc, mrun}, lane);
+      if constexpr (FOLD) {
+        const float4 v = ws.buf()[2 * K0 * 64 + 8];
+#pragma unroll
+        for (int q = 0; q < kNC; ++q) sc[q] = bound_scale(fmaf(v.y, m_in[q], v.z) + umax[q]);
+        op4<K0, 16, C16, false, false>(ws, OP(0), OP(1), Uh, Ul, xinv, pd, nopre,
+                                       FoldEpi4{Vh, Vl, sc, mrun, ufold}, lane);
+      } else {
+        next_scales(K0, sc);
+        op4<K0, 16, C16, false, false>(ws, OP(0), OP(1), Uh, Ul, xinv, pd, nopre, ReluEpi4{Vh, Vl, sc, mrun}, lane);
+      }
       finish(sc);
     }
     {
@@ -3201,11 +3254,13 @@
 
 int launch_sdf(const SdfLayout& L, const void* packed, const float* pts, int64_t P, float* sdf, float* nabla,
                float* feature, int nfreq, void* ws, size_t ws_bytes, hipStream_t stream, const int* P_dev,
-               int P_mult) {
+               int P_mult, const void* f8_alt) {
   if (P <= 0) return NR_OK;
   const int grid = grid_for(P);
+  NR_REQUIRE(!f8_alt || (feature && L.prec == NR_PREC_F16X3 && !L.siren), NR_ERR_ARG,
+             "sdf: an op in F8's place needs the f16x3 softplus net and a feature buffer");
   SdfKArgs a{(const char*)packed, L, pts, P, sdf, nabla, feature, (float4*)ws, nfreq, P_dev, P_mult, nullptr, nullptr,
-             nullptr};
+             nullptr, (const char*)f8_alt};
   ProfScope prof(nabla ? (feature ? "sdf_nabla_feat" : "sdf_nabla") : (feature ? "sdf_feat" : "sdf_fwd"), (double)P,
                  stream, P_dev, P_mult);
   if (L.siren) {
@@ -3339,10 +3394,13 @@
 
 int launch_radiance(const RadLayout& L, const void* packed, const float* x, const float* vdir, int64_t vdiv,
                     int64_t vmod, const float* normals, const float* feature, int64_t P, float* rgb, int nfreq_view,
-                    hipStream_t stream, const int* P_dev) {
+                    hipStream_t stream, const int* P_dev, const void* r0_fold) {
   if (P <= 0) return NR_OK;
   const int grid = grid_for(P);
-  RadKArgs a{(const char*)packed, L, x, vdir, vdiv, vmod, normals, feature, P, rgb, nfreq_view, P_dev};
+  NR_REQUIRE(!r0_fold || (L.prec == NR_PREC_F16X3 && !L.siren && L.D == 4), NR_ERR_ARG,
+             "radiance: the folded layer 0 needs the f16x3 ReLU D=4 net");
+  RadKArgs a{(const char*)packed, L, x, vdir, vdiv, vmod, normals, feature, P, rgb, nfreq_view, P_dev,
+             (const char*)r0_fold};
   ProfScope prof("radiance", (double)P, stream, P_dev, 1);
   const bool h3 = L.prec == NR_PREC_F16X3;
 #define NR_RAD_LAUNCH(KBS, ACT, D)                                                                            \
@@ -3357,8 +3415,11 @@
     return NR_ERR_UNSUPPORTED;
   }
   if (h3 && !L.siren && L.D == 4) {
-    if (L.kbs == 2) hipLaunchKernelGGL((rad4_kernel<2>), dim3(grid), dim3(kT4), 0, stream, a);
-    else hipLaunchKernelGGL((rad4_kernel<4>), dim3(grid), dim3(kT4), 0, stream, a);
+    if (r0_fold) {
+      if (L.kbs == 2) hipLaunchKernelGGL((rad4_kernel<2, true>), dim3(grid), dim3(kT4), 0, stream, a);
+      else hipLaunchKernelGGL((rad4_kernel<4, true>), dim3(grid), dim3(kT4), 0, stream, a);
+    } else if (L.kbs == 2) hipLaunchKernelGGL((rad4_kernel<2, false>), dim3(grid), dim3(kT4), 0, stream, a);
+    else hipLaunchKernelGGL((rad4_kernel<4, false>), dim3(grid), dim3(kT4), 0, stream, a);
   } else if (!L.siren && L.D == 4) {
     if (L.kbs == 2) NR_RAD_LAUNCH(2, ACT_RELU, 4); else NR_RAD_LAUNCH(4, ACT_RELU, 4);
   } else if (!L.siren && L.D == 5) {
diff --git a/neurecon_amd/frameworks/neus.py b/neurecon_amd/frameworks/neus.py
--- a/neurecon_amd/frameworks/neus.py
+++ b/neurecon_amd/frameworks/neus.py
@@ -78,7 +78,8 @@
                   near_bypass=None, far_bypass=None, detailed_output=True, show_progress=False, perturb=False,
                   fixed_s_recp=1 / 64., N_samples=64, N_importance=64, N_outside=0,
                   upsample_algo='official_solution', N_nograd_samples=2048, N_upsample_iters=4,
-                  skip_zero_alpha=True, defer_sample_nablas=True, max_workspace_gb=None, **dummy_kwargs):
+                  skip_zero_alpha=True, defer_sample_nablas=True, max_workspace_gb=None, fold_feature=True,
+                  **dummy_kwargs):
     L.require_gpu(rays_o, 'rays_o')
     if wants_graph(model):
         return _train_render(rays_o, rays_d, model, obj_bounding_radius=obj_bounding_radius, batched=batched,
@@ -132,6 +133,8 @@
     a.rays_o, a.rays_d, a.n_rays = L.ptr(ro), L.ptr(rd), n
     a.sdf, a.sdf_packed = ctypes.pointer(sdf_desc), L.ptr(sdf_packed)
     a.rad, a.rad_packed = ctypes.pointer(rad_desc), L.ptr(rad_packed)
+    fold_packed = model.radiance_net.nr_fold_packed(model.implicit_surface, dev) if fold_feature else None
+    a.fold_packed = L.ptr(fold_packed)
     a.s, a.s_dev = 0.0, L.ptr(s_dev)
     a.no_mid_skip = 0 if skip_zero_alpha else 1
     a.no_defer = 0 if defer_sample_nablas else 1
```

Measured after the change: 693,700, median of 6. 1.02x the previous value.
